# SegataLab/metamlst

Hardware: NVIDIA B200
Metric: aligned reads/s (score+pileup+consensus) (higher is better)
Workload: dtype int32/u8 (integer bit-plane arithmetic)

## Files before the change

include/mmlst.h:

```cpp
#ifndef MMLST_H
#define MMLST_H

#include <stddef.h>
#include <stdint.h>

#ifdef __cplusplus
extern "C" {
#endif

#define MMLST_VERSION 200

enum {
    MMLST_OK = 0,
    MMLST_E_ARG = -1,
    MMLST_E_CUDA = -2,
    MMLST_E_IO = -3,
    MMLST_E_BAM = -4,
    MMLST_E_UNSORTED = -5,
    MMLST_E_PAIRED = -6,
    MMLST_E_RANGE = -7,
    MMLST_E_NOMEM = -8
};

typedef struct mmlst_ctx mmlst_ctx;

const char* mmlst_last_error(void);
int mmlst_version(void);
int mmlst_device_count(void);

int mmlst_create(int device, mmlst_ctx** out);
void mmlst_destroy(mmlst_ctx* ctx);
void* mmlst_stream(mmlst_ctx* ctx);
int mmlst_sync(mmlst_ctx* ctx);

void* mmlst_pinned_alloc(size_t bytes);
void mmlst_pinned_free(void* p);

int mmlst_score_dev(const uint32_t* tid, const int16_t* as0, const uint8_t* xm3, const uint16_t* qlen,
                    const uint32_t* orig_idx, uint64_t n_rec, uint64_t idx_base,
                    const uint8_t* allow, const uint32_t* locus_of, uint32_t n_ref,
                    int minscore, int max_xm, int min_read_len,
                    int64_t* sum_as, uint32_t* n_hit, uint32_t* first_idx, uint64_t* counters, void* stream);

int mmlst_build_runs(const uint32_t* tid, uint64_t n_rec, uint32_t* run_tid, uint32_t* run_start, uint32_t* chunk_run,
                     uint32_t* n_runs);
int mmlst_score_runs_dev(const uint32_t* run_tid, const uint32_t* run_start, uint32_t n_runs, const uint32_t* chunk_run,
                         const int16_t* as0, const uint8_t* xm3, const uint16_t* qlen, const uint32_t* orig_idx,
                         uint64_t n_rec, uint64_t idx_base, const uint8_t* allow, uint32_t n_ref,
                         int minscore, int max_xm, int min_read_len,
                         int64_t* sum_as, uint32_t* n_hit, uint32_t* first_idx, uint64_t* counters, void* stream);
int mmlst_chunk_qlen(const uint16_t* qlen, uint64_t n_rec, uint16_t* chunk_qlen, int* uniform);
int mmlst_score_runs_qc_dev(const uint32_t* run_tid, const uint32_t* run_start, uint32_t n_runs, const uint32_t* chunk_run,
                            const uint16_t* chunk_qlen, const int16_t* as0, const uint8_t* xm3, const uint32_t* orig_idx,
                            uint64_t n_rec, uint64_t idx_base, const uint8_t* allow, uint32_t n_ref,
                            int minscore, int max_xm, int min_read_len,
                            int64_t* sum_as, uint32_t* n_hit, uint32_t* first_idx, uint64_t* counters, void* stream);
#define MMLST_SCORE_VARIANT_DEFAULT 6
int mmlst_set_score_variant(int variant);
#define MMLST_SCORE_L2_HINTS_DEFAULT 1
int mmlst_set_score_l2_hints(int on);
int mmlst_debug_timeline(uint64_t* dev_buf);
#define MMLST_SCORE_GRID_DEFAULT 8
int mmlst_set_score_grid_scale(int eighths);
int mmlst_as_untransform_dev(int16_t* as0, const uint8_t* xm3, uint64_t n, int coeff, void* stream);
int mmlst_expand_chunk_qlen_dev(const uint16_t* chunk_qlen, uint64_t n_rec, uint16_t* qlen, void* stream);
int mmlst_expand_runs_dev(const uint32_t* run_tid, const uint32_t* run_start, uint32_t n_runs, const uint32_t* chunk_run,
                          uint64_t n_rec, uint32_t* tid, void* stream);

uint64_t mmlst_coverage_table_slots(uint64_t n_names_upper_bound);
int mmlst_coverage_dev(const uint32_t* tid, const int16_t* as0, const uint8_t* xm3, const uint16_t* qlen,
                       const uint32_t* orig_idx, const uint64_t* qhash, uint64_t n_rec, uint64_t idx_base,
                       const uint8_t* allow, const uint32_t* locus_of, uint32_t n_ref, int minscore, int max_xm,
                       int min_read_len, void* table, uint64_t table_slots, uint64_t* cov, void* stream);

typedef struct {
    int32_t pos;
    uint32_t row_off;
    uint16_t reflen;
    int16_t as_named;
    uint8_t xm_named;
    uint8_t pad;
    uint16_t nw;
} mmlst_prec;

typedef struct {
    uint32_t rec_begin, rec_end;
    uint32_t col_base, contig_len;
    uint32_t plane_delta;
    uint32_t reserved[3];
} mmlst_chunk;

uint32_t mmlst_chunk_records(uint64_t n_rec);

int mmlst_pileup_dev(const mmlst_prec* recs, const uint32_t* planes,
                     const mmlst_chunk* chunks, uint32_t n_chunks, uint32_t max_row_words,
                     int minscore, int max_xm, uint32_t* counts, uint32_t total_cols, int impl, void* stream);

int mmlst_depth_cap(const uint32_t* tid, const int32_t* pos, const uint32_t* reflen, uint64_t n, uint32_t maxcnt,
                    uint32_t sentinel_nodes, uint8_t* admitted);

int mmlst_consensus_dev(const uint32_t* counts, const uint8_t* dbseq, const uint32_t* col_off, uint32_t n_loci,
                        uint32_t mincov, uint8_t* cons, uint32_t* holes, uint32_t* snps, void* stream);

#define MMLST_SELECT_WARP_DEFAULT 0
int mmlst_set_select_warp_finalize(int on);
#define MMLST_SELECT_CONSUME 1u
#define MMLST_SELECT_SCRATCH_CLEAN 2u
#define MMLST_SELECT_LOCAL 4u
int mmlst_select_dev(int64_t* sum_as, uint32_t* n_hit, uint32_t* first_idx, const uint32_t* locus_rows, const uint32_t* locus_start,
                     const uint32_t* allele_num, uint32_t n_ref, const uint32_t* species_of_locus, const uint32_t* genes_in_db,
                     uint32_t n_loci, uint32_t n_species, int penalty, int nloci_pct, const uint64_t* contig_start,
                     const uint32_t* ref_len, const uint64_t* db_off, uint32_t chunk_records, void* scratch, size_t scratch_bytes,
                     uint32_t* header, uint32_t* chosen_tid, uint32_t* chosen_species, uint32_t* col_off, uint64_t* db_start,
                     mmlst_chunk* chunks, uint32_t max_chunks, uint32_t flags, uint64_t* counters,
                     uint32_t* chosen_first , void* stream);
int mmlst_set_pdl(int on);
int mmlst_pileup_indirect_dev(const mmlst_prec* recs, const uint32_t* planes, const mmlst_chunk* chunks, const uint32_t* header,
                              uint32_t max_row_words, int minscore, int max_xm, uint32_t* counts, int impl, void* stream);
int mmlst_pileup_consensus_indirect_dev(const mmlst_prec* recs, const uint32_t* planes, const mmlst_chunk* chunks, const uint32_t* header,
                                        uint32_t max_row_words, int minscore, int max_xm, uint32_t* counts, const uint8_t* db_ascii,
                                        const uint64_t* db_start, const uint32_t* col_off, uint32_t max_loci, uint32_t mincov, uint8_t* cons,
                                        uint32_t* holes, uint32_t* snps, uint32_t flags, uint32_t* ticket, void* stream);
#define MMLST_CONSENSUS_CONSUME 1u
int mmlst_consensus_indirect_dev(uint32_t* counts, const uint8_t* db_ascii, const uint64_t* db_start, const uint32_t* col_off,
                                 uint32_t max_loci, const uint32_t* header, uint32_t mincov, uint8_t* cons, uint32_t* holes,
                                 uint32_t* snps, uint32_t flags, void* stream);

int mmlst_xchg_publish_dev(const void* block, uint32_t bytes, const uint64_t* peer_base, uint32_t rank, uint32_t world,
                           uint64_t half_stride, uint64_t slot_stride, uint64_t flag_off, const uint64_t* epoch, void* stream);
int mmlst_xchg_await_dev(void* local_base, uint32_t bytes, uint32_t world, uint64_t half_stride, uint64_t slot_stride,
                         uint64_t flag_off, void* out_all, uint64_t* epoch, uint32_t* ticket, uint32_t* status, void* stream);

typedef struct mmlst_comm mmlst_comm;
int mmlst_comm_unique_id(uint8_t* id128);
int mmlst_comm_create(const uint8_t* id128, int rank, int world, int device, mmlst_comm** out);
void mmlst_comm_destroy(mmlst_comm* comm);
int mmlst_allreduce(mmlst_comm* comm, int64_t* score_block, size_t score_words, uint32_t* first_idx, size_t n_ref, uint32_t* counts, size_t n_counts,
                    void* stream);

int mmlst_hamming_min_dev(const uint32_t* db_hi, const uint32_t* db_lo, const uint16_t* row_len, uint32_t n_rows,
                          uint32_t W, const uint32_t* q_hi, const uint32_t* q_lo, const uint16_t* q_len, uint32_t n_q,
                          const uint32_t* blocks, uint32_t n_blocks, uint32_t row_index_base,
                          unsigned long long* best, void* stream);
int mmlst_hamming_exact_dev(const uint32_t* db_hi, const uint32_t* db_lo, const uint16_t* row_len, uint32_t n_rows, uint32_t W,
                            const uint32_t* q_hi, const uint32_t* q_lo, const uint16_t* q_len, uint32_t n_q,
                            const uint32_t* blocks, uint32_t n_blocks, uint32_t row_index_base,
                            const uint32_t* xr_ids, const uint32_t* xr_x, const uint8_t* xr_bytes, uint32_t n_xr,
                            const uint32_t* xq_ids, const uint32_t* xq_x, const uint8_t* xq_bytes, uint32_t n_xq,
                            unsigned long long* best, void* stream);
int mmlst_hamming_min_dev2(const uint32_t* db_hi, const uint32_t* db_lo, const uint16_t* row_len, uint32_t n_rows,
                           uint32_t W, const uint32_t* q_hi, const uint32_t* q_lo, const uint16_t* q_len, uint32_t n_q,
                           const uint32_t* blocks, uint32_t n_blocks, uint32_t max_block_rows, uint32_t max_block_queries,
                           uint32_t row_index_base, unsigned long long* best, void* stream);

typedef struct {
    const uint8_t* bytes; uint64_t n_bytes;
    const uint64_t* table; uint32_t n_blocks;
    int32_t as_xm_coeff;
} mmlst_zstream;

typedef struct {
    const uint8_t* bytes; uint64_t n_bytes;
    const uint64_t* table; uint32_t n_blocks;
    const uint32_t* contig_block;
} mmlst_zpileup;

typedef struct {
    const uint32_t* tid; const int16_t* as0; const uint8_t* xm3; const uint16_t* qlen; const uint32_t* orig_idx;
    uint64_t n_rec;
    const mmlst_prec* p_recs;
    const uint32_t* planes; uint64_t n_prec; uint64_t n_plane_words; uint32_t max_row_words;
    const uint64_t* contig_start;
    uint32_t n_ref;
    uint32_t n_runs;
    const uint32_t* run_tid; const uint32_t* run_start; const uint32_t* chunk_run;
    const uint16_t* chunk_qlen;
    const mmlst_zstream* z;
    const mmlst_zpileup* zp;
} mmlst_soa;

typedef struct { int minscore, max_xm, min_read_len; } mmlst_score_params;

int mmlst_score(mmlst_ctx* ctx, const mmlst_soa* soa, const uint8_t* allow, const uint32_t* locus_of, uint32_t n_loci,
                const mmlst_score_params* prm, int64_t* sum_as, uint32_t* n_hit, uint32_t* first_idx, uint64_t* counters);

typedef struct {
    const uint32_t* locus_of; const uint32_t* allele_num; uint32_t n_ref;
    const uint32_t* species_of_locus; uint32_t n_loci;
    const uint32_t* genes_in_db; uint32_t n_species;
    const uint8_t* db_ascii; const uint64_t* db_off; const uint32_t* bam_ln;
} mmlst_index;
typedef struct { int minscore, max_xm, min_read_len, penalty, nloci_pct; uint32_t mincov; int pileup_impl; } mmlst_sample_params;
typedef struct {
    uint32_t n_chosen, error_bits, bad_len_tid, reserved;
    uint64_t total_reads, ignored_reads;
    uint32_t* chosen_tid; uint32_t* chosen_species; uint32_t* col_off;
    uint8_t* cons; uint64_t cons_capacity;
    uint32_t* holes; uint32_t* snps;
    int64_t* sum_as; uint32_t* n_hit; uint32_t* first_idx;
} mmlst_sample_result;
int mmlst_index_upload(mmlst_ctx* ctx, const mmlst_index* index);
int mmlst_sample(mmlst_ctx* ctx, const mmlst_soa* soa, const uint8_t* allow, const mmlst_sample_params* prm, mmlst_sample_result* res);

#define MMLST_COVERAGE_STREAM_RESIDENT 1u
int mmlst_coverage(mmlst_ctx* ctx, const mmlst_soa* soa, const uint64_t* qhash, const uint8_t* allow, const uint32_t* locus_of,
                   uint32_t n_loci, const mmlst_score_params* prm, uint32_t flags, uint64_t* cov);

int mmlst_pileup_consensus(mmlst_ctx* ctx, const mmlst_soa* soa, const uint32_t* chosen_tid, uint32_t n_loci,
                           const uint8_t* dbseq, const uint32_t* col_off, int minscore, int max_xm, uint32_t mincov,
                           int impl, uint32_t* counts, uint8_t* cons, uint32_t* holes, uint32_t* snps);

int mmlst_db_upload(mmlst_ctx* ctx, const uint32_t* db_hi, const uint32_t* db_lo, const uint16_t* row_len,
                    uint32_t n_rows, uint32_t W);
int mmlst_hamming_min(mmlst_ctx* ctx, const uint32_t* q_hi, const uint32_t* q_lo, const uint16_t* q_len, uint32_t n_q,
                      const uint32_t* blocks, uint32_t n_blocks, uint32_t* min_dist, uint32_t* argmin_row);
int mmlst_db_upload_x(mmlst_ctx* ctx, const uint32_t* db_hi, const uint32_t* db_lo, const uint16_t* row_len, uint32_t n_rows,
                      uint32_t W, const uint32_t* xr_ids, const uint32_t* xr_x, const uint8_t* xr_bytes, uint32_t n_xr);
int mmlst_hamming_min_x(mmlst_ctx* ctx, const uint32_t* q_hi, const uint32_t* q_lo, const uint16_t* q_len, uint32_t n_q,
                        const uint32_t* xq_ids, const uint32_t* xq_x, const uint8_t* xq_bytes, uint32_t n_xq,
                        const uint32_t* blocks, uint32_t n_blocks, uint32_t* min_dist, uint32_t* argmin_row);

size_t mmlst_hamming_tc_image_bytes(uint32_t n, uint32_t W, uint32_t tile_rows);
int mmlst_hamming_tc_expand_dev(const uint32_t* hi, const uint32_t* lo, const uint16_t* len, uint32_t n, uint32_t W, int db_tiled_layout,
                                uint32_t tile_rows, uint8_t* image, uint32_t* tile_maxlen, void* stream);
int mmlst_hamming_tc_search_dev(const uint8_t* q_image, const uint32_t* q_tile_maxlen, const uint16_t* q_len, uint32_t n_q,
                                const uint8_t* db_image, const uint32_t* db_tile_maxlen, const uint16_t* row_len, uint32_t n_rows,
                                uint32_t W, uint32_t row_index_base, unsigned long long* best, void* stream);

int mmlst_exact_match_dev(const uint32_t* db_hi, const uint32_t* db_lo, const uint16_t* row_len, uint32_t n_rows, uint32_t W,
                          const uint32_t* q_hi, const uint32_t* q_lo, const uint16_t* q_len, uint32_t n_q,
                          const uint32_t* blocks, uint32_t n_blocks, uint32_t max_block_rows, uint32_t row_index_base,
                          const uint32_t* row_key , const uint32_t* xr_ids, const uint8_t* xr_bytes, uint32_t n_xr,
                          const uint32_t* xq_ids, const uint8_t* xq_bytes, uint32_t n_xq, uint32_t* first_row, void* stream);
int mmlst_db_row_keys(mmlst_ctx* ctx, const uint32_t* row_key, uint32_t n_rows);
int mmlst_exact_match(mmlst_ctx* ctx, const uint32_t* q_hi, const uint32_t* q_lo, const uint16_t* q_len, uint32_t n_q,
                      const uint32_t* xq_ids, const uint8_t* xq_bytes, uint32_t n_xq,
                      const uint32_t* blocks, uint32_t n_blocks, uint32_t* first_row);

int mmlst_st_match_dev(const uint32_t* prof_start, const uint32_t* prof_allele, uint32_t n_st,
                       const uint32_t* q_alleles, const uint32_t* q_n, uint32_t l_max, uint32_t n_q,
                       uint32_t* count, uint32_t* best, uint32_t* n_best, uint32_t* out_idx, uint32_t max_out, void* stream);
int mmlst_profiles_upload(mmlst_ctx* ctx, const uint32_t* prof_start, const uint32_t* prof_allele, uint32_t n_st);
int mmlst_st_match(mmlst_ctx* ctx, const uint32_t* q_alleles, const uint32_t* q_n, uint32_t l_max, uint32_t n_q,
                   uint32_t* best, uint32_t* n_best, uint32_t* out_idx, uint32_t max_out);

int mmlst_inflate_raw(const uint8_t* in, size_t n, uint8_t* out, size_t out_capacity, size_t* produced);

typedef struct mmlst_bam mmlst_bam;
typedef struct {
    int minqual; uint32_t max_depth; uint32_t sentinel_nodes; int n_threads; int pinned; int assume_sorted;
    int want_qhash; int check_crc;
    int lenient_tags;
} mmlst_unpack_opts;
typedef struct {
    mmlst_soa soa;
    const uint64_t* qhash;
    const uint32_t* ref_len;
    const char* ref_names;
    const char* header_text;
    uint64_t n_dropped_by_cap, n_unmapped_flag;
    int presorted, minqual; uint32_t max_depth;
    double seconds[5];
    uint64_t n_untagged;
} mmlst_bam_info_t;
int mmlst_bam_unpack(const char* path, const mmlst_unpack_opts* opts , mmlst_bam** out);
int mmlst_bam_info(const mmlst_bam* bam, mmlst_bam_info_t* info);
void mmlst_bam_free(mmlst_bam* bam);

typedef struct mmlst_dev_bam mmlst_dev_bam;
typedef struct {
    const uint32_t* tid; const int16_t* as0; const uint8_t* xm3; const uint16_t* qlen; const uint32_t* orig_idx; const uint64_t* qhash;
    const uint32_t* run_tid; const uint32_t* run_start; const uint32_t* chunk_run; const uint16_t* chunk_qlen; uint32_t n_runs;
    const mmlst_prec* p_recs; const uint32_t* planes;
    uint64_t n_rec, n_prec, n_plane_words; uint32_t max_row_words;
    const uint64_t* contig_start;
    const uint32_t* ref_len;
    const char* ref_names;
    const char* header_text;
    uint32_t n_ref;
    uint64_t n_dropped_by_cap, n_unmapped_flag, n_bgzf_blocks, compressed_bytes, inflated_bytes;
    int presorted, minqual; uint32_t max_depth; int boundary_repairs;
    double seconds[8];
} mmlst_dev_bam_info_t;
int mmlst_bam_ingest(int device, const uint8_t* bam, size_t n_bytes, const mmlst_unpack_opts* opts, void* stream, mmlst_dev_bam** out);
int mmlst_dev_bam_info(const mmlst_dev_bam* bam, mmlst_dev_bam_info_t* info);
void mmlst_dev_bam_free(mmlst_dev_bam* bam);
int mmlst_ingest_trim(int device);

#ifdef __cplusplus
}
#endif
#endif
```

metamlst_b200/bam.py:

```python
from __future__ import annotations

import ctypes as C
import os
from typing import Optional

import numpy as np

from . import native, packing


class UnpackOpts(C.Structure):
    _fields_ = [("minqual", C.c_int), ("max_depth", C.c_uint32), ("sentinel_nodes", C.c_uint32), ("n_threads", C.c_int),
                ("pinned", C.c_int), ("assume_sorted", C.c_int), ("want_qhash", C.c_int), ("check_crc", C.c_int), ("lenient_tags", C.c_int)]


class BamInfo(C.Structure):
    _fields_ = [("soa", native.Soa), ("qhash", C.c_void_p), ("ref_len", C.c_void_p), ("ref_names", C.c_char_p),
                ("header_text", C.c_char_p), ("n_dropped_by_cap", C.c_uint64), ("n_unmapped_flag", C.c_uint64),
                ("presorted", C.c_int), ("minqual", C.c_int), ("max_depth", C.c_uint32), ("seconds", C.c_double * 5), ("n_untagged", C.c_uint64)]


class _Handle:
    def __init__(self, h):
        self.h = h

    def __del__(self):
        try:
            if self.h:
                native.lib().mmlst_bam_free(self.h)
                self.h = None
        except Exception:
            pass


def _view(addr: Optional[int], n: int, dtype) -> np.ndarray:
    dt = np.dtype(dtype)
    if not addr or n == 0:
        return np.zeros(0, dtype=dt)
    buf = (C.c_uint8 * (n * dt.itemsize)).from_address(addr)
    return np.frombuffer(buf, dtype=dt, count=n)


def unpack_bam(path: str, minqual: int = packing.DEFAULT_MINQUAL, max_depth: Optional[int] = packing.DEFAULT_MAX_DEPTH,
               presorted: bool = False, threads: int = 0, pinned: bool = True, want_qhash: bool = True,
               sentinel_nodes: int = 1, lenient_tags: bool = False) -> packing.SoaHost:
    lib = native.lib()
    o = UnpackOpts(int(minqual), int(max_depth or 0), int(sentinel_nodes), int(threads), 1 if pinned else 0,
                   1 if presorted else 0, 1 if want_qhash else 0, 1, 1 if lenient_tags else 0)
    h = C.c_void_p()
    native.check(lib.mmlst_bam_unpack(path.encode(), C.byref(o), C.byref(h)))
    keep = _Handle(h)
    info = BamInfo()
    native.check(lib.mmlst_bam_info(h, C.byref(info)))
    s = info.soa
    n, P, n_ref = int(s.n_rec), int(s.n_prec), int(s.n_ref)
    names = info.ref_names.decode("latin-1").split("\n") if n_ref else []
    soa = packing.SoaHost(
        names, _view(info.ref_len, n_ref, np.uint32).astype(np.int32),
        _view(s.tid, n, np.uint32), _view(s.as0, n, np.int16), _view(s.xm3, n, np.uint8), _view(s.qlen, n, np.uint16),
        _view(s.orig_idx, n, np.uint32) if s.orig_idx else None,
        _view(s.p_recs, P, packing.PREC_DTYPE), _view(s.planes, int(s.n_plane_words), np.uint32), int(s.max_row_words),
        _view(s.contig_start, n_ref + 1, np.uint64), int(info.minqual), int(info.max_depth), int(info.n_dropped_by_cap))
    if s.run_tid:
        nr = int(s.n_runs)
        soa.run_tid, soa.run_start = _view(s.run_tid, nr, np.uint32), _view(s.run_start, nr + 1, np.uint32)
        soa.chunk_run = _view(s.chunk_run, (n + 255) // 256, np.uint32)
        soa.chunk_qlen = _view(s.chunk_qlen, (n + 255) // 256, np.uint16) if s.chunk_qlen else None
        if nr > 0.125 * n:
            soa.run_tid = soa.run_start = soa.chunk_run = soa.chunk_qlen = None
    soa.qhash = _view(info.qhash, 2 * n, np.uint64).reshape(n, 2) if info.qhash else None
    soa.header_text = (info.header_text or b"").decode("latin-1")
    soa.unpack_seconds = dict(zip(("read", "inflate", "parse", "sort", "pack"), [float(x) for x in info.seconds]))
    soa.lenient, soa.n_untagged = bool(lenient_tags), int(info.n_untagged)
    soa._keep = (keep,)
    return soa


class DevBamInfo(C.Structure):
    _fields_ = [("tid", C.c_void_p), ("as0", C.c_void_p), ("xm3", C.c_void_p), ("qlen", C.c_void_p), ("orig_idx", C.c_void_p), ("qhash", C.c_void_p),
                ("run_tid", C.c_void_p), ("run_start", C.c_void_p), ("chunk_run", C.c_void_p), ("chunk_qlen", C.c_void_p), ("n_runs", C.c_uint32),
                ("p_recs", C.c_void_p), ("planes", C.c_void_p),
                ("n_rec", C.c_uint64), ("n_prec", C.c_uint64), ("n_plane_words", C.c_uint64), ("max_row_words", C.c_uint32),
                ("contig_start", C.c_void_p), ("ref_len", C.c_void_p), ("ref_names", C.c_char_p), ("header_text", C.c_char_p), ("n_ref", C.c_uint32),
                ("n_dropped_by_cap", C.c_uint64), ("n_unmapped_flag", C.c_uint64), ("n_bgzf_blocks", C.c_uint64), ("compressed_bytes", C.c_uint64),
                ("inflated_bytes", C.c_uint64), ("presorted", C.c_int), ("minqual", C.c_int), ("max_depth", C.c_uint32), ("boundary_repairs", C.c_int),
                ("seconds", C.c_double * 8)]


class _DevHandle:
    def __init__(self, h):
        self.h = h

    def __del__(self):
        try:
            if self.h:
                native.lib().mmlst_dev_bam_free(self.h)
                self.h = None
        except Exception:
            pass


class _DevArray:

    def __init__(self, addr: int, n: int, typestr: str, keep):
        self.__cuda_array_interface__ = {"shape": (n,), "typestr": typestr, "data": (addr, False), "version": 2, "strides": None}
        self._keep = keep


class PinnedPool:

    def __init__(self):
        import threading
        self._lock = threading.Lock()
        self._free = []

    def get(self, n: int):
        import torch
        with self._lock:
            best = None
            for i, t in enumerate(self._free):
                if t.numel() >= n and (best is None or t.numel() < self._free[best].numel()):
                    best = i
            if best is not None:
                return self._free.pop(best)
        return torch.empty(max(int(n * 1.25), 1 << 20), dtype=torch.uint8, pin_memory=torch.cuda.is_available())

    def put(self, t) -> None:
        base = getattr(t, "_pool_base", None)
        if base is not None:
            with self._lock:
                if len(self._free) < 16:
                    self._free.append(base)


POOL = PinnedPool()


def read_pinned(path: str, pool: Optional[PinnedPool] = None):
    import torch
    size = os.path.getsize(path)
    if pool is not None:
        base = pool.get(size)
    else:
        base = torch.empty(max(size, 1), dtype=torch.uint8, pin_memory=torch.cuda.is_available())
    with open(path, "rb") as fh:
        got = fh.readinto(memoryview(base.numpy())[:size]) if size else 0
    if got != size:
        raise IOError("short read on %s" % path)
    view = base[:size]
    if pool is not None:
        view._pool_base = base
    return view


def ingest_bam(source, device=0, minqual: int = packing.DEFAULT_MINQUAL, max_depth: Optional[int] = packing.DEFAULT_MAX_DEPTH,
               presorted: bool = False, want_qhash: bool = True, sentinel_nodes: int = 1, check_crc: bool = False):
    import torch
    from . import streams
    dev = torch.device("cuda", device) if isinstance(device, int) else torch.device(device)
    data = read_pinned(source) if isinstance(source, str) else source
    addr = data.data_ptr() if hasattr(data, "data_ptr") else data.ctypes.data
    nbytes = int(data.numel() if hasattr(data, "numel") else data.size)
    lib = native.lib()
    o = UnpackOpts(int(minqual), int(max_depth or 0), int(sentinel_nodes), 0, 1, 1 if presorted else 0, 1 if want_qhash else 0,
                  1 if check_crc else 0, 0)
    h = C.c_void_p()
    with torch.cuda.device(dev):
        stream = torch.cuda.current_stream(dev).cuda_stream
        native.check(lib.mmlst_bam_ingest(dev.index or 0, addr, nbytes, C.byref(o), stream, C.byref(h)))
    keep = _DevHandle(h)
    info = DevBamInfo()
    native.check(lib.mmlst_dev_bam_info(h, C.byref(info)))
    n, P, n_ref, nr = int(info.n_rec), int(info.n_prec), int(info.n_ref), int(info.n_runs)

    def t(addr_, count, typestr, dtype):
        if not addr_ or count == 0:
            return torch.zeros(0, dtype=dtype, device=dev)
        return torch.as_tensor(_DevArray(addr_, count, typestr, keep), device=dev)

    s = streams.DeviceStreams()
    s._keep = keep
    s.ref_names = info.ref_names.decode("latin-1").split("\n") if n_ref else []
    s.ref_lens = _view(info.ref_len, n_ref, np.uint32).astype(np.int32)
    s.header_text = (info.header_text or b"").decode("latin-1")
    s.minqual, s.max_depth, s.n_dropped = int(info.minqual), int(info.max_depth), int(info.n_dropped_by_cap)
    s.idx_base = 0
    s.tid, s.as0 = t(info.tid, n, "<i4", torch.int32), t(info.as0, n, "<i2", torch.int16)
    s.xm3, s.qlen = t(info.xm3, n, "|u1", torch.uint8), t(info.qlen, n, "<i2", torch.int16)
    s.orig_idx = t(info.orig_idx, n, "<i4", torch.int32) if info.orig_idx else None
    s.qhash = t(info.qhash, 2 * n, "<i8", torch.int64).view(n, 2) if (info.qhash and want_qhash) else None
    s.p_recs = t(info.p_recs, 4 * P, "<i4", torch.int32).view(P, 4)
    s.planes = t(info.planes, int(info.n_plane_words), "<i4", torch.int32)
    s.n_prec, s.max_row_words = P, int(info.max_row_words)
    s.contig_start = _view(info.contig_start, n_ref + 1, np.uint64).copy()
    s.run_tid = s.run_start = s.chunk_run = s.chunk_qlen = None
    if nr and nr <= 0.125 * n:
        s.run_tid, s.run_start = t(info.run_tid, nr, "<i4", torch.int32), t(info.run_start, nr + 1, "<i4", torch.int32)
        s.chunk_run = t(info.chunk_run, (n + 255) // 256, "<i4", torch.int32)
        s.chunk_qlen = t(info.chunk_qlen, (n + 255) // 256, "<i2", torch.int16) if info.chunk_qlen else None
    s.presorted = bool(info.presorted)
    s.ingest_seconds = dict(zip(("h2d", "inflate", "chain", "parse", "sort", "score_stream", "cap_compact", "pack"), [float(x) for x in info.seconds]))
    s.ingest_stats = {"bgzf_blocks": int(info.n_bgzf_blocks), "compressed_bytes": int(info.compressed_bytes), "inflated_bytes": int(info.inflated_bytes),
                      "boundary_repairs": int(info.boundary_repairs), "unmapped_flag": int(info.n_unmapped_flag)}
    return s
```

metamlst_b200/csrc/score_runs.cu:

```cuda
#include <stdlib.h>

#include "score_runs_kernels.cuh"


static int g_score_variant = -1;
static int score_variant() {
    if (g_score_variant < 0) {
        const char* e = getenv("MMLST_SCORE_VARIANT");
        g_score_variant = (e && e[0] >= '0' && e[0] <= '6' && !e[1]) ? e[0] - '0' : MMLST_SCORE_VARIANT_DEFAULT;
    }
    return g_score_variant;
}
extern "C" int mmlst_set_score_variant(int v) {
    const int prev = score_variant();
    if (v >= 0 && v <= 6) g_score_variant = v;
    return prev;
}

static int g_score_l2_hints = -1;
static int score_l2_hints() {
    if (g_score_l2_hints < 0) {
        const char* e = getenv("MMLST_SCORE_L2_HINTS");
        g_score_l2_hints = e ? (e[0] == '1') : MMLST_SCORE_L2_HINTS_DEFAULT;
    }
    return g_score_l2_hints;
}
extern "C" int mmlst_set_score_l2_hints(int on) {
    const int prev = score_l2_hints();
    if (on == 0 || on == 1) g_score_l2_hints = on;
    return prev;
}

static int g_score_grid8 = -1;
static int score_grid8() {
    if (g_score_grid8 < 0) {
        const char* e = getenv("MMLST_SCORE_GRID");
        const int v = e ? atoi(e) : 0;
        g_score_grid8 = (v >= 1 && v <= 64) ? v : MMLST_SCORE_GRID_DEFAULT;
    }
    return g_score_grid8;
}
extern "C" int mmlst_set_score_grid_scale(int eighths) {
    const int prev = score_grid8();
    if (eighths >= 1 && eighths <= 64) g_score_grid8 = eighths;
    return prev;
}

static int score_runs_launch(const uint32_t* run_tid, const uint32_t* run_start, uint32_t n_runs, const uint32_t* chunk_run,
                             const int16_t* as0, const uint8_t* xm3, const uint16_t* qlen, const uint16_t* chunk_qlen, const uint32_t* orig_idx,
                             uint64_t n_rec, uint64_t idx_base, const uint8_t* allow, uint32_t n_ref, int minscore,
                             int max_xm, int min_read_len, int64_t* sum_as, uint32_t* n_hit, uint32_t* first_idx,
                             uint64_t* counters, void* stream) {
    if (n_rec == 0) return MMLST_OK;
    if (!run_tid || !run_start || !chunk_run || !n_runs || !as0 || !xm3 || (!qlen && !chunk_qlen) || !allow || !sum_as || !n_hit || !first_idx || !counters) {
        mmlst_set_error("mmlst_score_runs_dev: null pointer");
        return MMLST_E_ARG;
    }
    if (n_rec >= 0xffffff00ull) { mmlst_set_error("mmlst_score_runs_dev: %llu records do not fit 32-bit run offsets", (unsigned long long)n_rec); return MMLST_E_RANGE; }
    if ((reinterpret_cast<uintptr_t>(as0) & 15) || (reinterpret_cast<uintptr_t>(xm3) & 7) || (!chunk_qlen && (reinterpret_cast<uintptr_t>(qlen) & 15)) ||
        (orig_idx && (reinterpret_cast<uintptr_t>(orig_idx) & 15))) {
        mmlst_set_error("mmlst_score_runs_dev: record arrays must be 16-byte aligned (as0/qlen/orig_idx), 8 (xm3)");
        return MMLST_E_ARG;
    }
    RunArgs a{run_tid, run_start, chunk_run, n_runs, as0, xm3, qlen, orig_idx, chunk_qlen, n_rec, idx_base, allow, n_ref, minscore, max_xm,
              min_read_len, reinterpret_cast<long long*>(sum_as), n_hit, first_idx, reinterpret_cast<unsigned long long*>(counters), score_l2_hints()};
    const uint64_t nchunks = n_rec >> 8;
    uint64_t want = (nchunks + 15) / 16;
    const int variant = score_variant();
    const cudaStream_t st = static_cast<cudaStream_t>(stream);
    const bool tma_ok = !orig_idx && !(reinterpret_cast<uintptr_t>(xm3) & 15);
    if (variant == 6 && tma_ok && chunk_qlen) {
        static int pair_resident_by_device[MMLST_MAX_DEVICES] = {0};
        int& pair_resident = pair_resident_by_device[mmlst_current_device()];
        const size_t smem = (kThreads / 32) * 2u * (4u * 768u + sizeof(uint64_t));
        if (!pair_resident) {
            CUDA_TRY(cudaFuncSetAttribute(score_runs_ring_pair_kernel, cudaFuncAttributeMaxDynamicSharedMemorySize, static_cast<int>(smem)));
            CUDA_TRY(cudaFuncSetAttribute(score_runs_ring_pair_kernel, cudaFuncAttributePreferredSharedMemoryCarveout, cudaSharedmemCarveoutMaxShared));
            int r = 0;
            if (cudaOccupancyMaxActiveBlocksPerMultiprocessor(&r, score_runs_ring_pair_kernel, kThreads, smem) != cudaSuccess || r < 1) r = 1;
            pair_resident = r;
        }
        const uint64_t cap = static_cast<uint64_t>(mmlst_num_sms()) * pair_resident * score_grid8() / 8;
        if (want > cap) want = cap;
        if (want < 1) want = 1;
        score_runs_ring_pair_kernel<<<static_cast<unsigned>(want), kThreads, smem, st>>>(a);
        CUDA_TRY(cudaGetLastError());
        return MMLST_OK;
    }
    if (variant >= 2 && tma_ok) {
        static int ring_resident_by_device[MMLST_MAX_DEVICES][4][8] = {{{0}}};
        int (&ring_resident)[4][8] = ring_resident_by_device[mmlst_current_device()];
        const int hint = a.l2_hints ? 1 : 0;
        const int q = (chunk_qlen ? 1 : 0) + 2 * hint;
        const int rv = variant == 6 ? 5 : variant;
        const RingCfg cfg = chunk_qlen ? (hint ? ring_config<true, true>(rv) : ring_config<true, false>(rv))
                                       : (hint ? ring_config<false, true>(rv) : ring_config<false, false>(rv));
        const size_t smem = (kThreads / 32) * static_cast<size_t>(cfg.ns) * (cfg.ch * (chunk_qlen ? 768u : 1280u) + sizeof(uint64_t));
        if (!ring_resident[q][rv]) {
            CUDA_TRY(cudaFuncSetAttribute(cfg.kern, cudaFuncAttributeMaxDynamicSharedMemorySize, static_cast<int>(smem)));
            CUDA_TRY(cudaFuncSetAttribute(cfg.kern, cudaFuncAttributePreferredSharedMemoryCarveout, cudaSharedmemCarveoutMaxShared));
            int r = 0;
            if (cudaOccupancyMaxActiveBlocksPerMultiprocessor(&r, cfg.kern, kThreads, smem) != cudaSuccess || r < 1) r = 1;
            ring_resident[q][rv] = r;
        }
        const uint64_t cap = static_cast<uint64_t>(mmlst_num_sms()) * ring_resident[q][rv];
        if (want > cap) want = cap;
        if (want < 1) want = 1;
        cfg.kern<<<static_cast<unsigned>(want), kThreads, smem, st>>>(a);
        CUDA_TRY(cudaGetLastError());
        return MMLST_OK;
    }
    static int resident_by_device[MMLST_MAX_DEVICES][8] = {{0}};
    int (&resident)[8] = resident_by_device[mmlst_current_device()];
    const int v = (orig_idx ? 1 : 0) + 2 * (variant == 1 ? 1 : 0) + (chunk_qlen ? 4 : 0);
    void (*const kerns[8])(const RunArgs) = {score_runs_kernel<false, false, false>, score_runs_kernel<true, false, false>,
                                             score_runs_kernel<false, true, false>, score_runs_kernel<true, true, false>,
                                             score_runs_kernel<false, false, true>, score_runs_kernel<true, false, true>,
                                             score_runs_kernel<false, true, true>, score_runs_kernel<true, true, true>};
    void (*kern)(const RunArgs) = kerns[v];
    if (!resident[v]) {
        if (cudaOccupancyMaxActiveBlocksPerMultiprocessor(&resident[v], kern, kThreads, 0) != cudaSuccess || resident[v] < 1) resident[v] = 3;
    }
    const uint64_t cap = static_cast<uint64_t>(mmlst_num_sms()) * resident[v];
    if (want > cap) want = cap;
    if (want < 1) want = 1;
    kern<<<static_cast<unsigned>(want), kThreads, 0, st>>>(a);
    CUDA_TRY(cudaGetLastError());
    return MMLST_OK;
}

extern "C" int mmlst_score_runs_dev(const uint32_t* run_tid, const uint32_t* run_start, uint32_t n_runs, const uint32_t* chunk_run,
                                    const int16_t* as0, const uint8_t* xm3, const uint16_t* qlen, const uint32_t* orig_idx,
                                    uint64_t n_rec, uint64_t idx_base, const uint8_t* allow, uint32_t n_ref, int minscore,
                                    int max_xm, int min_read_len, int64_t* sum_as, uint32_t* n_hit, uint32_t* first_idx,
                                    uint64_t* counters, void* stream) {
    if (n_rec && !qlen) { mmlst_set_error("mmlst_score_runs_dev: null pointer"); return MMLST_E_ARG; }
    return score_runs_launch(run_tid, run_start, n_runs, chunk_run, as0, xm3, qlen, nullptr, orig_idx, n_rec, idx_base, allow, n_ref, minscore,
                             max_xm, min_read_len, sum_as, n_hit, first_idx, counters, stream);
}

extern "C" int mmlst_score_runs_qc_dev(const uint32_t* run_tid, const uint32_t* run_start, uint32_t n_runs, const uint32_t* chunk_run,
                                       const uint16_t* chunk_qlen, const int16_t* as0, const uint8_t* xm3, const uint32_t* orig_idx,
                                       uint64_t n_rec, uint64_t idx_base, const uint8_t* allow, uint32_t n_ref, int minscore,
                                       int max_xm, int min_read_len, int64_t* sum_as, uint32_t* n_hit, uint32_t* first_idx,
                                       uint64_t* counters, void* stream) {
    if (n_rec && !chunk_qlen) { mmlst_set_error("mmlst_score_runs_qc_dev: null pointer"); return MMLST_E_ARG; }
    return score_runs_launch(run_tid, run_start, n_runs, chunk_run, as0, xm3, nullptr, chunk_qlen, orig_idx, n_rec, idx_base, allow, n_ref,
                             minscore, max_xm, min_read_len, sum_as, n_hit, first_idx, counters, stream);
}

extern "C" int mmlst_expand_chunk_qlen_dev(const uint16_t* chunk_qlen, uint64_t n_rec, uint16_t* qlen, void* stream) {
    if (n_rec == 0) return MMLST_OK;
    if (!chunk_qlen || !qlen) { mmlst_set_error("mmlst_expand_chunk_qlen_dev: null pointer"); return MMLST_E_ARG; }
    uint64_t blocks = (n_rec + 255) / 256;
    const uint64_t cap = static_cast<uint64_t>(mmlst_num_sms()) * 16;
    if (blocks > cap) blocks = cap;
    expand_chunk_qlen_kernel<<<static_cast<unsigned>(blocks), 256, 0, static_cast<cudaStream_t>(stream)>>>(chunk_qlen, n_rec, qlen);
    CUDA_TRY(cudaGetLastError());
    return MMLST_OK;
}

extern "C" int mmlst_expand_runs_dev(const uint32_t* run_tid, const uint32_t* run_start, uint32_t n_runs, const uint32_t* chunk_run,
                                     uint64_t n_rec, uint32_t* tid, void* stream) {
    if (n_rec == 0) return MMLST_OK;
    if (!run_tid || !run_start || !chunk_run || !n_runs || !tid) { mmlst_set_error("mmlst_expand_runs_dev: null pointer"); return MMLST_E_ARG; }
    uint64_t blocks = (n_rec + 255) / 256;
    const uint64_t cap = static_cast<uint64_t>(mmlst_num_sms()) * 16;
    if (blocks > cap) blocks = cap;
    expand_runs_kernel<<<static_cast<unsigned>(blocks), 256, 0, static_cast<cudaStream_t>(stream)>>>(run_tid, run_start, chunk_run, n_runs, n_rec, tid);
    CUDA_TRY(cudaGetLastError());
    return MMLST_OK;
}

namespace {
__global__ void __launch_bounds__(256) as_untransform_kernel(int16_t* __restrict__ as0, const uint8_t* __restrict__ xm3, uint64_t n, int coeff) {
    const uint64_t n8 = n >> 3;
    const uint64_t stride = static_cast<uint64_t>(gridDim.x) * blockDim.x;
    for (uint64_t i = static_cast<uint64_t>(blockIdx.x) * blockDim.x + threadIdx.x; i < n8; i += stride) {
        uint4 a = reinterpret_cast<uint4*>(as0)[i];
        const uint2 x = ld_stream_u2(xm3 + (i << 3));
        uint32_t aw[4] = {a.x, a.y, a.z, a.w};
        const uint32_t xw[2] = {x.x, x.y};
#pragma unroll
        for (int w = 0; w < 4; ++w) {
            const uint32_t xb = xw[w >> 1] >> ((w & 1) * 16);
            const int lo = static_cast<int16_t>(aw[w] & 0xffffu) - coeff * static_cast<int>(xb & 0xffu);
            const int hi = static_cast<int16_t>(aw[w] >> 16) - coeff * static_cast<int>((xb >> 8) & 0xffu);
            aw[w] = (static_cast<uint32_t>(lo) & 0xffffu) | (static_cast<uint32_t>(hi) << 16);
        }
        reinterpret_cast<uint4*>(as0)[i] = make_uint4(aw[0], aw[1], aw[2], aw[3]);
    }
    if (blockIdx.x == 0 && threadIdx.x == 0)
        for (uint64_t i = n8 << 3; i < n; ++i) as0[i] = static_cast<int16_t>(as0[i] - coeff * static_cast<int>(xm3[i]));
}
}

extern "C" int mmlst_as_untransform_dev(int16_t* as0, const uint8_t* xm3, uint64_t n, int coeff, void* stream) {
    if (n == 0 || coeff == 0) return MMLST_OK;
    if (!as0 || !xm3) { mmlst_set_error("mmlst_as_untransform_dev: null pointer"); return MMLST_E_ARG; }
    if ((reinterpret_cast<uintptr_t>(as0) & 15) || (reinterpret_cast<uintptr_t>(xm3) & 7)) { mmlst_set_error("mmlst_as_untransform_dev: as0 must be 16-byte aligned, xm3 8"); return MMLST_E_ARG; }
    uint64_t blocks = ((n >> 3) + 255) / 256;
    const uint64_t cap = static_cast<uint64_t>(mmlst_num_sms()) * 8;
    if (blocks > cap) blocks = cap;
    if (blocks < 1) blocks = 1;
    as_untransform_kernel<<<static_cast<unsigned>(blocks), 256, 0, static_cast<cudaStream_t>(stream)>>>(as0, xm3, n, coeff);
    CUDA_TRY(cudaGetLastError());
    return MMLST_OK;
}
```

metamlst_b200/csrc/score_runs_kernels.cuh:

```cuda
#pragma once
#include "common.cuh"

namespace {

constexpr int kThreads = 256;
constexpr uint32_t FULL = 0xffffffffu;

struct RunArgs {
    const uint32_t* run_tid; const uint32_t* run_start; const uint32_t* chunk_run; uint32_t n_runs;
    const int16_t* as0; const uint8_t* xm3; const uint16_t* qlen; const uint32_t* orig_idx;
    const uint16_t* chunk_qlen;
    uint64_t n_rec; uint64_t idx_base;
    const uint8_t* allow; uint32_t n_ref;
    int minscore, max_xm, min_read_len;
    long long* sum_as; uint32_t* n_hit; uint32_t* first_idx; unsigned long long* counters;
    int l2_hints;
};

__device__ __forceinline__ void flush_run(const RunArgs& a, uint32_t key, long long s, uint32_t c, uint32_t mn) {
    if (c) {
        atomicAdd(reinterpret_cast<unsigned long long*>(a.sum_as + key), static_cast<unsigned long long>(s));
        atomicAdd(a.n_hit + key, c);
        atomicMin(a.first_idx + key, mn);
    }
}

template <bool OIDX> struct Loaded;
template <> struct Loaded<false> { uint4 a8, q8; uint2 x8; uint32_t cq; };
template <> struct Loaded<true> { uint4 a8, q8; uint2 x8; uint32_t cq; uint4 oa, ob; };

template <bool OIDX, bool QC>
__device__ __forceinline__ Loaded<OIDX> load_chunk(const RunArgs& a, uint64_t base_lane) {
    Loaded<OIDX> L;
    L.a8 = ld_stream_u4(a.as0 + base_lane);
    L.x8 = ld_stream_u2(a.xm3 + base_lane);
    if constexpr (QC) { L.cq = __ldg(a.chunk_qlen + (base_lane >> 8)); L.q8 = make_uint4(0, 0, 0, 0); }
    else { L.q8 = ld_stream_u4(a.qlen + base_lane); L.cq = 0; }
    if constexpr (OIDX) { L.oa = ld_stream_u4(a.orig_idx + base_lane); L.ob = ld_stream_u4(a.orig_idx + base_lane + 4); }
    return L;
}

template <bool OIDX>
__device__ __forceinline__ uint32_t rec_index(const Loaded<OIDX>& L, uint32_t idx0, int k) {
    if constexpr (OIDX) {
        const uint32_t oi[8] = {L.oa.x, L.oa.y, L.oa.z, L.oa.w, L.ob.x, L.ob.y, L.ob.z, L.ob.w};
        return oi[k];
    } else {
        return idx0 + k;
    }
}

struct WarpRun {
    uint32_t r, key, end;
    bool al;
    long long s; uint32_t c, mn;
};

__device__ __forceinline__ void open_run(const RunArgs& a, WarpRun& w, uint32_t r) {
    w.r = r;
    if (r < a.n_runs) {
        w.key = __ldg(a.run_tid + r);
        w.end = __ldg(a.run_start + r + 1);
        w.al = (w.key < a.n_ref) && a.allow[w.key];
    } else {
        w.key = 0xffffffffu; w.end = 0xffffffffu; w.al = false;
    }
    w.s = 0; w.c = 0; w.mn = 0xffffffffu;
}

__device__ __forceinline__ void close_run(const RunArgs& a, WarpRun& w, uint32_t lane) {
    if (lane == 0 && w.al) flush_run(a, w.key, w.s, w.c, w.mn);
}

struct Thr {
    uint32_t as_T, as_TL;
    uint32_t ql_T, ql_TL;
    uint32_t xm_T, xm_TH;
    uint32_t h8;
};
constexpr uint32_t H16 = 0x80008000u, H8 = 0x80808080u;

__device__ __forceinline__ Thr make_thr(const RunArgs& a) {
    Thr t;
    const bool none = a.minscore > 32767 || a.min_read_len > 65535 || a.max_xm < 0;
    const uint32_t ts = static_cast<uint32_t>(max(a.minscore, -32768) + 32768) & 0xffffu;
    const uint32_t tq = static_cast<uint32_t>(min(max(a.min_read_len, 0), 65535));
    const uint32_t tx = static_cast<uint32_t>(min(max(a.max_xm, 0), 255));
    t.as_T = ts | (ts << 16); t.as_TL = t.as_T & ~H16;
    t.ql_T = tq | (tq << 16); t.ql_TL = t.ql_T & ~H16;
    t.xm_T = tx * 0x01010101u; t.xm_TH = t.xm_T | H8;
    t.h8 = none ? 0u : H8;
    return t;
}

template <bool OIDX, bool QC>
__device__ __forceinline__ void lane_pass(const Loaded<OIDX>& L, const Thr& t, int min_read_len, uint32_t& p_lo, uint32_t& p_hi) {
    const uint32_t aw[4] = {L.a8.x, L.a8.y, L.a8.z, L.a8.w};
    const uint32_t qw[4] = {L.q8.x, L.q8.y, L.q8.z, L.q8.w};
    uint32_t m[4];
#pragma unroll
    for (int w = 0; w < 4; ++w) {
        const uint32_t da = (aw[w] | H16) - t.as_TL;
        const uint32_t ga = (~aw[w] & ~t.as_T) | ((aw[w] ^ t.as_T) & da);
        if constexpr (QC) {
            m[w] = ga;
        } else {
            const uint32_t dq = (qw[w] | H16) - t.ql_TL;
            const uint32_t gq = (qw[w] & ~t.ql_T) | (~(qw[w] ^ t.ql_T) & dq);
            m[w] = ga & gq;
        }
    }
    const uint32_t b_lo = __byte_perm(m[0], m[1], 0x7531), b_hi = __byte_perm(m[2], m[3], 0x7531);
    const uint32_t x0 = L.x8.x, x1 = L.x8.y;
    const uint32_t d0 = t.xm_TH - (x0 & ~H8), d1 = t.xm_TH - (x1 & ~H8);
    const uint32_t g0 = (t.xm_T & ~x0) | (~(t.xm_T ^ x0) & d0), g1 = (t.xm_T & ~x1) | (~(t.xm_T ^ x1) & d1);
    p_lo = (b_lo & g0 & t.h8) >> 7;
    p_hi = (b_hi & g1 & t.h8) >> 7;
    if constexpr (QC) {
        if (static_cast<int>(L.cq) < min_read_len) { p_lo = 0; p_hi = 0; }
    }
}

template <bool OIDX>
__device__ __forceinline__ void lane_sums(const Loaded<OIDX>& L, uint32_t p_lo, uint32_t p_hi, uint32_t idx0, int& s, uint32_t& c, uint32_t& mn) {
    s = __dp2a_lo(static_cast<int>(L.a8.x), static_cast<int>(p_lo), 0);
    s = __dp2a_hi(static_cast<int>(L.a8.y), static_cast<int>(p_lo), s);
    s = __dp2a_lo(static_cast<int>(L.a8.z), static_cast<int>(p_hi), s);
    s = __dp2a_hi(static_cast<int>(L.a8.w), static_cast<int>(p_hi), s);
    c = __popc(p_lo | (p_hi << 1));
    if constexpr (OIDX) {
        mn = 0xffffffffu;
#pragma unroll
        for (int k = 0; k < 8; ++k) mn = (((k < 4 ? p_lo : p_hi) >> (8 * (k & 3))) & 1u) ? min(mn, rec_index<true>(L, idx0, k)) : mn;
    } else {
        const uint32_t k = p_lo ? (static_cast<uint32_t>(__ffs(p_lo)) - 1u) >> 3 : 4u + ((static_cast<uint32_t>(__ffs(p_hi)) - 1u) >> 3);
        mn = (p_lo | p_hi) ? idx0 + k : 0xffffffffu;
    }
}

template <bool OIDX, bool QC>
__device__ __forceinline__ void reduce_chunk(const RunArgs& a, const Thr& thr, WarpRun& w, const Loaded<OIDX>& L, uint64_t base, uint32_t lane,
                                             uint32_t& tot, uint32_t& ign) {
    constexpr uint32_t R = 8;
    const uint64_t rec0 = base + (lane << 3);
    const uint32_t idx0 = static_cast<uint32_t>(a.idx_base + rec0);
    uint32_t p_lo, p_hi;
    lane_pass<OIDX, QC>(L, thr, a.min_read_len, p_lo, p_hi);
    const uint64_t chunk_end = base + 256;
    if (chunk_end <= w.end) {
        if (w.al) {
            int s; uint32_t c, mn;
            lane_sums<OIDX>(L, p_lo, p_hi, idx0, s, c, mn);
            tot += R;
            ign += R - c;
            w.s += __reduce_add_sync(FULL, s);
            w.c += __reduce_add_sync(FULL, c);
            w.mn = min(w.mn, __reduce_min_sync(FULL, mn));
        }
        if (chunk_end == w.end) { close_run(a, w, lane); open_run(a, w, w.r + 1); }
        return;
    }
    uint64_t lo = base;
    while (lo < chunk_end) {
        const uint64_t hi = (w.end < chunk_end) ? static_cast<uint64_t>(w.end) : chunk_end;
        if (w.al) {
            const uint32_t klo = lo <= rec0 ? 0u : (lo - rec0 >= R ? R : static_cast<uint32_t>(lo - rec0));
            const uint32_t khi = hi <= rec0 ? 0u : (hi - rec0 >= R ? R : static_cast<uint32_t>(hi - rec0));
            const unsigned long long ones = 0x0101010101010101ull;
            const unsigned long long below_hi = khi >= 8 ? ~0ull : ((1ull << (8 * khi)) - 1ull);
            const unsigned long long below_lo = klo >= 8 ? ~0ull : ((1ull << (8 * klo)) - 1ull);
            const unsigned long long inm = khi > klo ? (below_hi & ~below_lo & ones) : 0ull;
            const uint32_t in_lo = static_cast<uint32_t>(inm), in_hi = static_cast<uint32_t>(inm >> 32);
            int s; uint32_t c, mn;
            lane_sums<OIDX>(L, p_lo & in_lo, p_hi & in_hi, idx0, s, c, mn);
            const uint32_t in = khi > klo ? khi - klo : 0u;
            tot += in;
            ign += in - c;
            w.s += __reduce_add_sync(FULL, s);
            w.c += __reduce_add_sync(FULL, c);
            w.mn = min(w.mn, __reduce_min_sync(FULL, mn));
        }
        if (hi == w.end) { close_run(a, w, lane); open_run(a, w, w.r + 1); }
        lo = hi;
    }
}

template <bool QC>
__device__ __forceinline__ void score_tail(const RunArgs& a, uint64_t nchunks, uint32_t lane, uint32_t& tot, uint32_t& ign) {
    uint32_t r = __ldg(a.chunk_run + nchunks);
    for (uint64_t i = (nchunks << 8) + lane; i < a.n_rec; i += 32) {
        while (r + 1 < a.n_runs && i >= a.run_start[r + 1]) ++r;
        const uint32_t key = a.run_tid[r];
        if (!((key < a.n_ref) && a.allow[key])) continue;
        ++tot;
        const int as = a.as0[i];
        const int ql = QC ? int(a.chunk_qlen[nchunks]) : int(a.qlen[i]);
        if ((as >= a.minscore) && (ql >= a.min_read_len) && (int(a.xm3[i]) <= a.max_xm)) {
            const uint32_t idx = a.orig_idx ? a.orig_idx[i] : static_cast<uint32_t>(a.idx_base + i);
            flush_run(a, key, as, 1u, idx);
        } else {
            ++ign;
        }
    }
}

template <bool OIDX, bool PIPE, bool QC>
__global__ void __launch_bounds__(kThreads, PIPE ? (OIDX ? 2 : 3) : (OIDX ? 3 : 4)) score_runs_kernel(const RunArgs a) {
    pdl_launch_dependents();
    const uint32_t lane = threadIdx.x & 31u;
    const uint64_t warp = (static_cast<uint64_t>(blockIdx.x) * blockDim.x + threadIdx.x) >> 5;
    const uint64_t nwarps = (static_cast<uint64_t>(gridDim.x) * blockDim.x) >> 5;
    const uint64_t nchunks = a.n_rec >> 8;
    const uint64_t per = (nchunks + nwarps - 1) / nwarps;
    const uint64_t c0 = warp * per;
    const uint64_t c1 = (c0 + per < nchunks) ? c0 + per : nchunks;
    uint32_t tot = 0, ign = 0;
    const Thr thr = make_thr(a);

    if (c0 < c1) {
        uint64_t ch = c0;
        Loaded<OIDX> A0, A1;
        bool have = ch + 1 < c1;
        if (have) { A0 = load_chunk<OIDX, QC>(a, (ch << 8) + (lane << 3)); A1 = load_chunk<OIDX, QC>(a, ((ch + 1) << 8) + (lane << 3)); }
        WarpRun w;
        open_run(a, w, __ldg(a.chunk_run + c0));
        Loaded<OIDX> B0, B1;
        if constexpr (!PIPE) {
            while (have) {
                reduce_chunk<OIDX, QC>(a, thr, w, A0, ch << 8, lane, tot, ign);
                reduce_chunk<OIDX, QC>(a, thr, w, A1, (ch + 1) << 8, lane, tot, ign);
                ch += 2;
                have = ch + 1 < c1;
                if (have) { A0 = load_chunk<OIDX, QC>(a, (ch << 8) + (lane << 3)); A1 = load_chunk<OIDX, QC>(a, ((ch + 1) << 8) + (lane << 3)); }
            }
        }
        while (have) {
            const bool moreB = ch + 3 < c1;
            if (moreB) { B0 = load_chunk<OIDX, QC>(a, ((ch + 2) << 8) + (lane << 3)); B1 = load_chunk<OIDX, QC>(a, ((ch + 3) << 8) + (lane << 3)); }
            reduce_chunk<OIDX, QC>(a, thr, w, A0, ch << 8, lane, tot, ign);
            reduce_chunk<OIDX, QC>(a, thr, w, A1, (ch + 1) << 8, lane, tot, ign);
            ch += 2;
            if (!moreB) break;
            have = ch + 3 < c1;
            if (have) { A0 = load_chunk<OIDX, QC>(a, ((ch + 2) << 8) + (lane << 3)); A1 = load_chunk<OIDX, QC>(a, ((ch + 3) << 8) + (lane << 3)); }
            reduce_chunk<OIDX, QC>(a, thr, w, B0, ch << 8, lane, tot, ign);
            reduce_chunk<OIDX, QC>(a, thr, w, B1, (ch + 1) << 8, lane, tot, ign);
            ch += 2;
        }
        if (ch < c1) {
            const uint64_t base = ch << 8;
            const Loaded<OIDX> L0 = load_chunk<OIDX, QC>(a, base + (lane << 3));
            reduce_chunk<OIDX, QC>(a, thr, w, L0, base, lane, tot, ign);
        }
        close_run(a, w, lane);
    }

    if (warp == nwarps - 1 && (a.n_rec & 255u)) score_tail<QC>(a, nchunks, lane, tot, ign);
    tot = __reduce_add_sync(FULL, tot);
    ign = __reduce_add_sync(FULL, ign);
    if (lane == 0 && tot) {
        atomicAdd(a.counters + 0, static_cast<unsigned long long>(tot));
        atomicAdd(a.counters + 1, static_cast<unsigned long long>(ign));
    }
}

struct WarpRunPF {
    uint32_t r, key, end;
    uint32_t nkey, nend;
    bool al;
    long long s; uint32_t c, mn;
};

template <bool HINT> __device__ __forceinline__ uint32_t tab_u32(const uint32_t* p, uint64_t pol) {
    if constexpr (HINT) return ld_table_u32(p, pol); else return __ldg(p);
}
template <bool HINT> __device__ __forceinline__ uint32_t tab_u16(const uint16_t* p, uint64_t pol) {
    if constexpr (HINT) return ld_table_u16(p, pol); else return __ldg(p);
}
template <bool HINT> __device__ __forceinline__ uint32_t tab_u8(const uint8_t* p, uint64_t pol) {
    if constexpr (HINT) return ld_table_u8(p, pol); else return *p;
}
template <bool HINT>
__device__ __forceinline__ void request_next_run(const RunArgs& a, WarpRunPF& w, uint64_t pol) {
    if (w.r + 1u < a.n_runs) { w.nkey = tab_u32<HINT>(a.run_tid + w.r + 1u, pol); w.nend = tab_u32<HINT>(a.run_start + w.r + 2u, pol); }
    else { w.nkey = 0xffffffffu; w.nend = 0xffffffffu; }
}
template <bool HINT>
__device__ __forceinline__ void open_run_pf(const RunArgs& a, WarpRunPF& w, uint32_t r, uint64_t pol) {
    w.r = r;
    if (r < a.n_runs) { w.key = tab_u32<HINT>(a.run_tid + r, pol); w.end = tab_u32<HINT>(a.run_start + r + 1u, pol); }
    else { w.key = 0xffffffffu; w.end = 0xffffffffu; }
    request_next_run<HINT>(a, w, pol);
    w.al = (w.key < a.n_ref) && tab_u8<HINT>(a.allow + w.key, pol);
    w.s = 0; w.c = 0; w.mn = 0xffffffffu;
}
template <bool HINT>
__device__ __forceinline__ void next_run_pf(const RunArgs& a, WarpRunPF& w, uint32_t lane, uint64_t pol) {
    if (lane == 0 && w.al) flush_run(a, w.key, w.s, w.c, w.mn);
    w.r += 1u; w.key = w.nkey; w.end = w.nend;
    request_next_run<HINT>(a, w, pol);
    w.al = (w.key < a.n_ref) && tab_u8<HINT>(a.allow + w.key, pol);
    w.s = 0; w.c = 0; w.mn = 0xffffffffu;
}

__device__ __forceinline__ uint32_t bytes_below(uint32_t k) { return k >= 4u ? 0xffffffffu : ((1u << (8u * k)) - 1u); }
__device__ __forceinline__ void segment_masks(uint32_t klo, uint32_t khi, uint32_t& in_lo, uint32_t& in_hi) {
    in_lo = bytes_below(min(khi, 4u)) & ~bytes_below(min(klo, 4u)) & 0x01010101u;
    in_hi = bytes_below(khi > 4u ? khi - 4u : 0u) & ~bytes_below(klo > 4u ? klo - 4u : 0u) & 0x01010101u;
}

__device__ __forceinline__ void lane_sums_pf(const Loaded<false>& L, uint32_t p_lo, uint32_t p_hi, int& s, uint32_t& c) {
    s = __dp2a_lo(static_cast<int>(L.a8.x), static_cast<int>(p_lo), 0);
    s = __dp2a_hi(static_cast<int>(L.a8.y), static_cast<int>(p_lo), s);
    s = __dp2a_lo(static_cast<int>(L.a8.z), static_cast<int>(p_hi), s);
    s = __dp2a_hi(static_cast<int>(L.a8.w), static_cast<int>(p_hi), s);
    c = __popc(p_lo | (p_hi << 1));
}
__device__ __forceinline__ uint32_t first_pass_index(uint32_t p_lo, uint32_t p_hi, uint32_t idx0) {
    const uint32_t k = p_lo ? (static_cast<uint32_t>(__ffs(p_lo)) - 1u) >> 3 : 4u + ((static_cast<uint32_t>(__ffs(p_hi)) - 1u) >> 3);
    return (p_lo | p_hi) ? idx0 + k : 0xffffffffu;
}

template <bool QC, bool HINT>
__device__ __forceinline__ void reduce_chunk_pf(const RunArgs& a, const Thr& thr, WarpRunPF& w, const Loaded<false>& L, uint32_t base, uint32_t lane,
                                                uint32_t& tot, uint32_t& ign, uint64_t pol) {
    constexpr uint32_t R = 8;
    const uint32_t idx0 = static_cast<uint32_t>(a.idx_base) + base + (lane << 3);
    uint32_t p_lo, p_hi;
    lane_pass<false, QC>(L, thr, a.min_read_len, p_lo, p_hi);
    const uint32_t chunk_end = base + 256u;
    if (chunk_end <= w.end) {
        if (w.al) {
            int s; uint32_t c;
            lane_sums_pf(L, p_lo, p_hi, s, c);
            tot += R;
            ign += R - c;
            w.s += __reduce_add_sync(FULL, s);
            w.c += __reduce_add_sync(FULL, c);
            if (w.mn == 0xffffffffu) w.mn = __reduce_min_sync(FULL, first_pass_index(p_lo, p_hi, idx0));
        }
        if (chunk_end == w.end) next_run_pf<HINT>(a, w, lane, pol);
        return;
    }
    const int lane0 = static_cast<int>(lane << 3);
    uint32_t lo = base;
    while (lo < chunk_end) {
        const uint32_t hi = min(w.end, chunk_end);
        if (w.al) {
            const uint32_t klo = static_cast<uint32_t>(min(max(static_cast<int>(lo - base) - lane0, 0), 8));
            const uint32_t khi = static_cast<uint32_t>(min(max(static_cast<int>(hi - base) - lane0, 0), 8));
            uint32_t in_lo, in_hi;
            segment_masks(klo, khi, in_lo, in_hi);
            int s; uint32_t c;
            lane_sums_pf(L, p_lo & in_lo, p_hi & in_hi, s, c);
            const uint32_t in = khi - klo;
            tot += in;
            ign += in - c;
            w.s += __reduce_add_sync(FULL, s);
            w.c += __reduce_add_sync(FULL, c);
            if (w.mn == 0xffffffffu) w.mn = __reduce_min_sync(FULL, first_pass_index(p_lo & in_lo, p_hi & in_hi, idx0));
        }
        if (hi == w.end) next_run_pf<HINT>(a, w, lane, pol);
        lo = hi;
    }
}

template <bool QC, int NS, int CH, int MINB, bool HINT>
__global__ void __launch_bounds__(kThreads, MINB) score_runs_ring_kernel(const RunArgs a) {
    pdl_launch_dependents();
    extern __shared__ __align__(128) uint8_t ring_raw[];
    constexpr uint32_t AS_B = CH * 512u, QL_B = QC ? 0u : CH * 512u, XM_B = CH * 256u;
    constexpr uint32_t STAGE_B = AS_B + QL_B + XM_B;
    constexpr uint32_t CH_B = STAGE_B / CH;
    constexpr int NW = kThreads / 32;
    const uint32_t lane = threadIdx.x & 31u, wid = threadIdx.x >> 5;
    uint8_t* const my = ring_raw + wid * (NS * STAGE_B);
    uint64_t* const bars = reinterpret_cast<uint64_t*>(ring_raw + NW * NS * STAGE_B) + wid * NS;
    if (threadIdx.x == 0) {
        uint64_t* all = reinterpret_cast<uint64_t*>(ring_raw + NW * NS * STAGE_B);
        for (int i = 0; i < NW * NS; ++i) mbar_init(all + i, 1);
        fence_mbar_init();
    }
    __syncthreads();

    const uint64_t warp = (static_cast<uint64_t>(blockIdx.x) * blockDim.x + threadIdx.x) >> 5;
    const uint64_t nwarps = (static_cast<uint64_t>(gridDim.x) * blockDim.x) >> 5;
    const uint64_t nchunks = a.n_rec >> 8;
    const uint64_t per = (nchunks + nwarps - 1) / nwarps;
    const uint64_t c0 = warp * per;
    const uint64_t c1 = (c0 + per < nchunks) ? c0 + per : nchunks;
    uint32_t tot = 0, ign = 0;
    const Thr thr = make_thr(a);
    const uint64_t pol_s = HINT ? l2_policy(1) : 0ull, pol_t = HINT ? l2_policy(2) : 0ull;

    if (c0 < c1) {
        const uint32_t ngroups = static_cast<uint32_t>((c1 - c0 + CH - 1) / CH);
        auto issue = [&](uint32_t g, int stage) {
            const uint64_t ch = c0 + static_cast<uint64_t>(g) * CH;
            const uint32_t nch = (c1 - ch < CH) ? static_cast<uint32_t>(c1 - ch) : static_cast<uint32_t>(CH);
            uint8_t* st = my + stage * STAGE_B;
            mbar_expect_tx(bars + stage, nch * CH_B);
            if constexpr (HINT) {
                bulk_g2s_hint(st, a.as0 + (ch << 8), nch * 512u, bars + stage, pol_s);
                if constexpr (!QC) bulk_g2s_hint(st + AS_B, a.qlen + (ch << 8), nch * 512u, bars + stage, pol_s);
                bulk_g2s_hint(st + AS_B + QL_B, a.xm3 + (ch << 8), nch * 256u, bars + stage, pol_s);
            } else {
                bulk_g2s(st, a.as0 + (ch << 8), nch * 512u, bars + stage);
                if constexpr (!QC) bulk_g2s(st + AS_B, a.qlen + (ch << 8), nch * 512u, bars + stage);
                bulk_g2s(st + AS_B + QL_B, a.xm3 + (ch << 8), nch * 256u, bars + stage);
            }
        };
        if (lane == 0) {
            const uint32_t pre = ngroups < static_cast<uint32_t>(NS) ? ngroups : static_cast<uint32_t>(NS);
            for (uint32_t g = 0; g < pre; ++g) issue(g, static_cast<int>(g));
        }
        WarpRunPF w;
        open_run_pf<HINT>(a, w, tab_u32<HINT>(a.chunk_run + c0, pol_t), pol_t);
        uint32_t phase = 0;
        int stage = 0;
        for (uint32_t g = 0; g < ngroups; ++g) {
            const uint64_t ch = c0 + static_cast<uint64_t>(g) * CH;
            const uint32_t nch = (c1 - ch < CH) ? static_cast<uint32_t>(c1 - ch) : static_cast<uint32_t>(CH);
            mbar_wait(bars + stage, (phase >> stage) & 1u);
            phase ^= 1u << stage;
            const uint8_t* st = my + stage * STAGE_B;
#pragma unroll
            for (uint32_t k = 0; k < static_cast<uint32_t>(CH); ++k) {
                if (k < nch) {
                    Loaded<false> L;
                    L.a8 = *reinterpret_cast<const uint4*>(st + k * 512u + lane * 16u);
                    L.x8 = *reinterpret_cast<const uint2*>(st + AS_B + QL_B + k * 256u + lane * 8u);
                    if constexpr (QC) { L.q8 = make_uint4(0, 0, 0, 0); L.cq = tab_u16<HINT>(a.chunk_qlen + ch + k, pol_t); }
                    else { L.q8 = *reinterpret_cast<const uint4*>(st + AS_B + k * 512u + lane * 16u); L.cq = 0; }
                    if (k + 1u == nch) {
                        __syncwarp();
                        if (lane == 0 && g + NS < ngroups) issue(g + NS, stage);
                    }
                    reduce_chunk_pf<QC, HINT>(a, thr, w, L, static_cast<uint32_t>((ch + k) << 8), lane, tot, ign, pol_t);
                }
            }
            stage = (stage + 1 == NS) ? 0 : stage + 1;
        }
        if (lane == 0 && w.al) flush_run(a, w.key, w.s, w.c, w.mn);
    }

    if (warp == nwarps - 1 && (a.n_rec & 255u)) score_tail<QC>(a, nchunks, lane, tot, ign);
    tot = __reduce_add_sync(FULL, tot);
    ign = __reduce_add_sync(FULL, ign);
    if (lane == 0 && tot) {
        atomicAdd(a.counters + 0, static_cast<unsigned long long>(tot));
        atomicAdd(a.counters + 1, static_cast<unsigned long long>(ign));
    }
}

__device__ __forceinline__ void reduce_pair_pf(const RunArgs& a, const Thr& thr, WarpRunPF& w, const Loaded<false>& La, const Loaded<false>& Lb,
                                               uint32_t base, uint32_t lane, uint32_t& tot, uint32_t& ign, uint64_t pol) {
    if (base + 512u > w.end) {
        reduce_chunk_pf<true, false>(a, thr, w, La, base, lane, tot, ign, pol);
        reduce_chunk_pf<true, false>(a, thr, w, Lb, base + 256u, lane, tot, ign, pol);
        return;
    }
    if (w.al) {
        uint32_t pa_lo, pa_hi, pb_lo, pb_hi;
        lane_pass<false, true>(La, thr, a.min_read_len, pa_lo, pa_hi);
        lane_pass<false, true>(Lb, thr, a.min_read_len, pb_lo, pb_hi);
        int s = __dp2a_lo(static_cast<int>(La.a8.x), static_cast<int>(pa_lo), 0);
        s = __dp2a_hi(static_cast<int>(La.a8.y), static_cast<int>(pa_lo), s);
        s = __dp2a_lo(static_cast<int>(La.a8.z), static_cast<int>(pa_hi), s);
        s = __dp2a_hi(static_cast<int>(La.a8.w), static_cast<int>(pa_hi), s);
        s = __dp2a_lo(static_cast<int>(Lb.a8.x), static_cast<int>(pb_lo), s);
        s = __dp2a_hi(static_cast<int>(Lb.a8.y), static_cast<int>(pb_lo), s);
        s = __dp2a_lo(static_cast<int>(Lb.a8.z), static_cast<int>(pb_hi), s);
        s = __dp2a_hi(static_cast<int>(Lb.a8.w), static_cast<int>(pb_hi), s);
        const uint32_t c = __popc(pa_lo | (pa_hi << 1) | (pb_lo << 2) | (pb_hi << 3));
        tot += 16u;
        ign += 16u - c;
        w.s += __reduce_add_sync(FULL, s);
        w.c += __reduce_add_sync(FULL, c);
        if (w.mn == 0xffffffffu) {
            const uint32_t idx0 = static_cast<uint32_t>(a.idx_base) + base + (lane << 3);
            const uint32_t ma = first_pass_index(pa_lo, pa_hi, idx0);
            w.mn = __reduce_min_sync(FULL, ma != 0xffffffffu ? ma : first_pass_index(pb_lo, pb_hi, idx0 + 256u));
        }
    }
    if (base + 512u == w.end) next_run_pf<false>(a, w, lane, pol);
}

__global__ void __launch_bounds__(kThreads, 4) score_runs_ring_pair_kernel(const RunArgs a) {
    pdl_launch_dependents();
    extern __shared__ __align__(128) uint8_t ring_raw[];
    constexpr int NS = 2;
    constexpr uint32_t CH = 4, AS_B = CH * 512u, XM_B = CH * 256u, STAGE_B = AS_B + XM_B, CH_B = STAGE_B / CH;
    constexpr int NW = kThreads / 32;
    const uint32_t lane = threadIdx.x & 31u, wid = threadIdx.x >> 5;
    uint8_t* const my = ring_raw + wid * (NS * STAGE_B);
    uint64_t* const bars = reinterpret_cast<uint64_t*>(ring_raw + NW * NS * STAGE_B) + wid * NS;
    if (threadIdx.x == 0) {
        uint64_t* all = reinterpret_cast<uint64_t*>(ring_raw + NW * NS * STAGE_B);
        for (int i = 0; i < NW * NS; ++i) mbar_init(all + i, 1);
        fence_mbar_init();
    }
    __syncthreads();

    const uint64_t warp = (static_cast<uint64_t>(blockIdx.x) * blockDim.x + threadIdx.x) >> 5;
    const uint64_t nwarps = (static_cast<uint64_t>(gridDim.x) * blockDim.x) >> 5;
    const uint64_t nchunks = a.n_rec >> 8;
    const uint64_t per = (nchunks + nwarps - 1) / nwarps;
    const uint64_t c0 = warp * per;
    const uint64_t c1 = (c0 + per < nchunks) ? c0 + per : nchunks;
    uint32_t tot = 0, ign = 0;
    const Thr thr = make_thr(a);

    if (c0 < c1) {
        const uint32_t ngroups = static_cast<uint32_t>((c1 - c0 + CH - 1) / CH);
        auto issue = [&](uint32_t g, int stage) {
            const uint64_t ch = c0 + static_cast<uint64_t>(g) * CH;
            const uint32_t nch = (c1 - ch < CH) ? static_cast<uint32_t>(c1 - ch) : CH;
            uint8_t* st = my + stage * STAGE_B;
            mbar_expect_tx(bars + stage, nch * CH_B);
            if (a.l2_hints) {
                const uint64_t pol_s = l2_policy(1);
                bulk_g2s_hint(st, a.as0 + (ch << 8), nch * 512u, bars + stage, pol_s);
                bulk_g2s_hint(st + AS_B, a.xm3 + (ch << 8), nch * 256u, bars + stage, pol_s);
            } else {
                bulk_g2s(st, a.as0 + (ch << 8), nch * 512u, bars + stage);
                bulk_g2s(st + AS_B, a.xm3 + (ch << 8), nch * 256u, bars + stage);
            }
        };
        if (lane == 0) {
            const uint32_t pre = ngroups < static_cast<uint32_t>(NS) ? ngroups : static_cast<uint32_t>(NS);
            for (uint32_t g = 0; g < pre; ++g) issue(g, static_cast<int>(g));
        }
        WarpRunPF w;
        open_run_pf<false>(a, w, __ldg(a.chunk_run + c0), 0ull);
        uint32_t phase = 0;
        int stage = 0;
        auto load = [&](const uint8_t* st, uint32_t k, uint64_t ch) {
            Loaded<false> L;
            L.a8 = *reinterpret_cast<const uint4*>(st + k * 512u + lane * 16u);
            L.x8 = *reinterpret_cast<const uint2*>(st + AS_B + k * 256u + lane * 8u);
            L.q8 = make_uint4(0, 0, 0, 0);
            L.cq = __ldg(a.chunk_qlen + ch + k);
            return L;
        };
        for (uint32_t g = 0; g < ngroups; ++g) {
            const uint64_t ch = c0 + static_cast<uint64_t>(g) * CH;
            const uint32_t nch = (c1 - ch < CH) ? static_cast<uint32_t>(c1 - ch) : CH;
            mbar_wait(bars + stage, (phase >> stage) & 1u);
            phase ^= 1u << stage;
            const uint8_t* st = my + stage * STAGE_B;
#pragma unroll
            for (uint32_t k = 0; k < CH; k += 2) {
                if (k < nch) {
                    const bool two = k + 1u < nch;
                    const Loaded<false> La = load(st, k, ch);
                    Loaded<false> Lb = La;
                    if (two) Lb = load(st, k + 1u, ch);
                    if (k + 2u >= nch) {
                        __syncwarp();
                        if (lane == 0 && g + NS < ngroups) issue(g + NS, stage);
                    }
                    const uint32_t base = static_cast<uint32_t>((ch + k) << 8);
                    if (two) reduce_pair_pf(a, thr, w, La, Lb, base, lane, tot, ign, 0ull);
                    else reduce_chunk_pf<true, false>(a, thr, w, La, base, lane, tot, ign, 0ull);
                }
            }
            stage = (stage + 1 == NS) ? 0 : stage + 1;
        }
        if (lane == 0 && w.al) flush_run(a, w.key, w.s, w.c, w.mn);
    }

    if (warp == nwarps - 1 && (a.n_rec & 255u)) score_tail<true>(a, nchunks, lane, tot, ign);
    tot = __reduce_add_sync(FULL, tot);
    ign = __reduce_add_sync(FULL, ign);
    if (lane == 0 && tot) {
        atomicAdd(a.counters + 0, static_cast<unsigned long long>(tot));
        atomicAdd(a.counters + 1, static_cast<unsigned long long>(ign));
    }
}

struct RingCfg { void (*kern)(const RunArgs); uint32_t ch, ns; };
template <bool QC, bool HINT>
inline RingCfg ring_config(int variant) {
    if constexpr (QC) {
        switch (variant) {
            case 3: return {score_runs_ring_kernel<true, 3, 4, 3, HINT>, 4, 3};
            case 4: return {score_runs_ring_kernel<true, 2, 8, 2, HINT>, 8, 2};
            case 5: return {score_runs_ring_kernel<true, 2, 4, 4, HINT>, 4, 2};
            default: return {score_runs_ring_kernel<true, 4, 2, 4, HINT>, 2, 4};
        }
    } else {
        switch (variant) {
            case 3: case 4: case 5: return {score_runs_ring_kernel<false, 2, 4, 2, HINT>, 4, 2};
            default: return {score_runs_ring_kernel<false, 3, 2, 3, HINT>, 2, 3};
        }
    }
}

__global__ void __launch_bounds__(256) expand_runs_kernel(const uint32_t* __restrict__ run_tid, const uint32_t* __restrict__ run_start,
                                                          const uint32_t* __restrict__ chunk_run, uint32_t n_runs, uint64_t n_rec,
                                                          uint32_t* __restrict__ tid) {
    const uint64_t stride = static_cast<uint64_t>(gridDim.x) * blockDim.x;
    for (uint64_t i = static_cast<uint64_t>(blockIdx.x) * blockDim.x + threadIdx.x; i < n_rec; i += stride) {
        uint32_t r = __ldg(chunk_run + (i >> 8));
        while (r + 1 < n_runs && i >= __ldg(run_start + r + 1)) ++r;
        tid[i] = __ldg(run_tid + r);
    }
}

__global__ void __launch_bounds__(256) expand_chunk_qlen_kernel(const uint16_t* __restrict__ chunk_qlen, uint64_t n_rec, uint16_t* __restrict__ qlen) {
    const uint64_t stride = static_cast<uint64_t>(gridDim.x) * blockDim.x;
    for (uint64_t i = static_cast<uint64_t>(blockIdx.x) * blockDim.x + threadIdx.x; i < n_rec; i += stride) qlen[i] = __ldg(chunk_qlen + (i >> 8));
}

}
```

metamlst_b200/native.py:

```python
from __future__ import annotations

import ctypes as C
import os

_HERE = os.path.dirname(os.path.abspath(__file__))
LIB_PATH = os.path.join(_HERE, "libmmlst.so")


class MmlstError(RuntimeError):
    def __init__(self, code: int, msg: str):
        super().__init__("libmmlst error %d: %s" % (code, msg))
        self.code = code


E_ARG, E_CUDA, E_IO, E_BAM, E_UNSORTED, E_PAIRED, E_RANGE, E_NOMEM = -1, -2, -3, -4, -5, -6, -7, -8


class Chunk(C.Structure):
    _fields_ = [("rec_begin", C.c_uint32), ("rec_end", C.c_uint32), ("col_base", C.c_uint32), ("contig_len", C.c_uint32),
                ("plane_delta", C.c_uint32), ("reserved", C.c_uint32 * 3)]


class Soa(C.Structure):
    _fields_ = [("tid", C.c_void_p), ("as0", C.c_void_p), ("xm3", C.c_void_p), ("qlen", C.c_void_p), ("orig_idx", C.c_void_p),
                ("n_rec", C.c_uint64),
                ("p_recs", C.c_void_p),
                ("planes", C.c_void_p), ("n_prec", C.c_uint64), ("n_plane_words", C.c_uint64), ("max_row_words", C.c_uint32),
                ("contig_start", C.c_void_p), ("n_ref", C.c_uint32),
                ("n_runs", C.c_uint32), ("run_tid", C.c_void_p), ("run_start", C.c_void_p), ("chunk_run", C.c_void_p),
                ("chunk_qlen", C.c_void_p), ("z", C.c_void_p), ("zp", C.c_void_p)]


class ZStream(C.Structure):
    _fields_ = [("bytes", C.c_void_p), ("n_bytes", C.c_uint64), ("table", C.c_void_p), ("n_blocks", C.c_uint32), ("as_xm_coeff", C.c_int32)]


class ZPileup(C.Structure):
    _fields_ = [("bytes", C.c_void_p), ("n_bytes", C.c_uint64), ("table", C.c_void_p), ("n_blocks", C.c_uint32), ("contig_block", C.c_void_p)]


class ScoreParams(C.Structure):
    _fields_ = [("minscore", C.c_int), ("max_xm", C.c_int), ("min_read_len", C.c_int)]


class Index(C.Structure):
    _fields_ = [("locus_of", C.c_void_p), ("allele_num", C.c_void_p), ("n_ref", C.c_uint32),
                ("species_of_locus", C.c_void_p), ("n_loci", C.c_uint32),
                ("genes_in_db", C.c_void_p), ("n_species", C.c_uint32),
                ("db_ascii", C.c_void_p), ("db_off", C.c_void_p), ("bam_ln", C.c_void_p)]


class SampleParams(C.Structure):
    _fields_ = [("minscore", C.c_int), ("max_xm", C.c_int), ("min_read_len", C.c_int), ("penalty", C.c_int), ("nloci_pct", C.c_int),
                ("mincov", C.c_uint32), ("pileup_impl", C.c_int)]


class SampleResult(C.Structure):
    _fields_ = [("n_chosen", C.c_uint32), ("error_bits", C.c_uint32), ("bad_len_tid", C.c_uint32), ("reserved", C.c_uint32),
                ("total_reads", C.c_uint64), ("ignored_reads", C.c_uint64),
                ("chosen_tid", C.c_void_p), ("chosen_species", C.c_void_p), ("col_off", C.c_void_p),
                ("cons", C.c_void_p), ("cons_capacity", C.c_uint64),
                ("holes", C.c_void_p), ("snps", C.c_void_p),
                ("sum_as", C.c_void_p), ("n_hit", C.c_void_p), ("first_idx", C.c_void_p)]


EXPORTS = {
    "mmlst_last_error": (C.c_char_p, []),
    "mmlst_version": (C.c_int, []),
    "mmlst_device_count": (C.c_int, []),
    "mmlst_create": (C.c_int, [C.c_int, C.POINTER(C.c_void_p)]),
    "mmlst_destroy": (None, [C.c_void_p]),
    "mmlst_stream": (C.c_void_p, [C.c_void_p]),
    "mmlst_sync": (C.c_int, [C.c_void_p]),
    "mmlst_pinned_alloc": (C.c_void_p, [C.c_size_t]),
    "mmlst_pinned_free": (None, [C.c_void_p]),
    "mmlst_score_dev": (C.c_int, [C.c_void_p] * 5 + [C.c_uint64, C.c_uint64, C.c_void_p, C.c_void_p, C.c_uint32,
                                  C.c_int, C.c_int, C.c_int, C.c_void_p, C.c_void_p, C.c_void_p, C.c_void_p, C.c_void_p]),
    "mmlst_build_runs": (C.c_int, [C.c_void_p, C.c_uint64, C.c_void_p, C.c_void_p, C.c_void_p, C.POINTER(C.c_uint32)]),
    "mmlst_score_runs_dev": (C.c_int, [C.c_void_p, C.c_void_p, C.c_uint32] + [C.c_void_p] * 5 + [C.c_uint64, C.c_uint64, C.c_void_p, C.c_uint32,
                                       C.c_int, C.c_int, C.c_int, C.c_void_p, C.c_void_p, C.c_void_p, C.c_void_p, C.c_void_p]),
    "mmlst_chunk_qlen": (C.c_int, [C.c_void_p, C.c_uint64, C.c_void_p, C.POINTER(C.c_int)]),
    "mmlst_score_runs_qc_dev": (C.c_int, [C.c_void_p, C.c_void_p, C.c_uint32] + [C.c_void_p] * 5 + [C.c_uint64, C.c_uint64, C.c_void_p, C.c_uint32,
                                          C.c_int, C.c_int, C.c_int, C.c_void_p, C.c_void_p, C.c_void_p, C.c_void_p, C.c_void_p]),
    "mmlst_expand_chunk_qlen_dev": (C.c_int, [C.c_void_p, C.c_uint64, C.c_void_p, C.c_void_p]),
    "mmlst_inflate_raw": (C.c_int, [C.c_void_p, C.c_size_t, C.c_void_p, C.c_size_t, C.POINTER(C.c_size_t)]),
    "mmlst_set_score_variant": (C.c_int, [C.c_int]),
    "mmlst_set_score_l2_hints": (C.c_int, [C.c_int]),
    "mmlst_set_score_grid_scale": (C.c_int, [C.c_int]),
    "mmlst_debug_timeline": (C.c_int, [C.c_void_p]),
    "mmlst_set_select_warp_finalize": (C.c_int, [C.c_int]),
    "mmlst_as_untransform_dev": (C.c_int, [C.c_void_p, C.c_void_p, C.c_uint64, C.c_int, C.c_void_p]),
    "mmlst_set_pdl": (C.c_int, [C.c_int]),
    "mmlst_expand_runs_dev": (C.c_int, [C.c_void_p, C.c_void_p, C.c_uint32, C.c_void_p, C.c_uint64, C.c_void_p, C.c_void_p]),
    "mmlst_coverage_table_slots": (C.c_uint64, [C.c_uint64]),
    "mmlst_coverage_dev": (C.c_int, [C.c_void_p] * 6 + [C.c_uint64, C.c_uint64, C.c_void_p, C.c_void_p, C.c_uint32, C.c_int, C.c_int,
                                     C.c_int, C.c_void_p, C.c_uint64, C.c_void_p, C.c_void_p]),
    "mmlst_coverage": (C.c_int, [C.c_void_p, C.POINTER(Soa), C.c_void_p, C.c_void_p, C.c_void_p, C.c_uint32, C.POINTER(ScoreParams),
                                 C.c_uint32, C.c_void_p]),
    "mmlst_pileup_dev": (C.c_int, [C.c_void_p] * 3 + [C.c_uint32, C.c_uint32, C.c_int, C.c_int, C.c_void_p, C.c_uint32,
                                   C.c_int, C.c_void_p]),
    "mmlst_consensus_dev": (C.c_int, [C.c_void_p, C.c_void_p, C.c_void_p, C.c_uint32, C.c_uint32, C.c_void_p, C.c_void_p,
                                      C.c_void_p, C.c_void_p]),
    "mmlst_hamming_min_dev": (C.c_int, [C.c_void_p, C.c_void_p, C.c_void_p, C.c_uint32, C.c_uint32, C.c_void_p, C.c_void_p,
                                        C.c_void_p, C.c_uint32, C.c_void_p, C.c_uint32, C.c_uint32, C.c_void_p, C.c_void_p]),
    "mmlst_hamming_min_dev2": (C.c_int, [C.c_void_p, C.c_void_p, C.c_void_p, C.c_uint32, C.c_uint32, C.c_void_p, C.c_void_p,
                                         C.c_void_p, C.c_uint32, C.c_void_p, C.c_uint32, C.c_uint32, C.c_uint32, C.c_uint32,
                                         C.c_void_p, C.c_void_p]),
    "mmlst_select_dev": (C.c_int, [C.c_void_p] * 6 + [C.c_uint32, C.c_void_p, C.c_void_p, C.c_uint32, C.c_uint32, C.c_int, C.c_int,
                                   C.c_void_p, C.c_void_p, C.c_void_p, C.c_uint32, C.c_void_p, C.c_size_t] + [C.c_void_p] * 6 +
                         [C.c_uint32, C.c_uint32, C.c_void_p, C.c_void_p, C.c_void_p]),
    "mmlst_pileup_indirect_dev": (C.c_int, [C.c_void_p] * 4 + [C.c_uint32, C.c_int, C.c_int, C.c_void_p, C.c_int, C.c_void_p]),
    "mmlst_consensus_indirect_dev": (C.c_int, [C.c_void_p] * 4 + [C.c_uint32, C.c_void_p, C.c_uint32, C.c_void_p, C.c_void_p, C.c_void_p,
                                                C.c_uint32, C.c_void_p]),
    "mmlst_pileup_consensus_indirect_dev": (C.c_int, [C.c_void_p] * 4 + [C.c_uint32, C.c_int, C.c_int, C.c_void_p, C.c_void_p, C.c_void_p, C.c_void_p, C.c_uint32,
                                                      C.c_uint32, C.c_void_p, C.c_void_p, C.c_void_p, C.c_uint32, C.c_void_p, C.c_void_p]),
    "mmlst_chunk_records": (C.c_uint32, [C.c_uint64]),
    "mmlst_xchg_publish_dev": (C.c_int, [C.c_void_p, C.c_uint32, C.c_void_p, C.c_uint32, C.c_uint32, C.c_uint64, C.c_uint64, C.c_uint64,
                                         C.c_void_p, C.c_void_p]),
    "mmlst_xchg_await_dev": (C.c_int, [C.c_void_p, C.c_uint32, C.c_uint32, C.c_uint64, C.c_uint64, C.c_uint64, C.c_void_p, C.c_void_p,
                                       C.c_void_p, C.c_void_p, C.c_void_p]),
    "mmlst_depth_cap": (C.c_int, [C.c_void_p, C.c_void_p, C.c_void_p, C.c_uint64, C.c_uint32, C.c_uint32, C.c_void_p]),
    "mmlst_score": (C.c_int, [C.c_void_p, C.POINTER(Soa), C.c_void_p, C.c_void_p, C.c_uint32, C.POINTER(ScoreParams),
                              C.c_void_p, C.c_void_p, C.c_void_p, C.c_void_p]),
    "mmlst_pileup_consensus": (C.c_int, [C.c_void_p, C.POINTER(Soa), C.c_void_p, C.c_uint32, C.c_void_p, C.c_void_p, C.c_int,
                                         C.c_int, C.c_uint32, C.c_int, C.c_void_p, C.c_void_p, C.c_void_p, C.c_void_p]),
    "mmlst_db_upload": (C.c_int, [C.c_void_p, C.c_void_p, C.c_void_p, C.c_void_p, C.c_uint32, C.c_uint32]),
    "mmlst_db_upload_x": (C.c_int, [C.c_void_p, C.c_void_p, C.c_void_p, C.c_void_p, C.c_uint32, C.c_uint32, C.c_void_p, C.c_void_p,
                                    C.c_void_p, C.c_uint32]),
    "mmlst_hamming_min_x": (C.c_int, [C.c_void_p, C.c_void_p, C.c_void_p, C.c_void_p, C.c_uint32, C.c_void_p, C.c_void_p, C.c_void_p,
                                      C.c_uint32, C.c_void_p, C.c_uint32, C.c_void_p, C.c_void_p]),
    "mmlst_hamming_exact_dev": (C.c_int, [C.c_void_p, C.c_void_p, C.c_void_p, C.c_uint32, C.c_uint32, C.c_void_p, C.c_void_p, C.c_void_p,
                                          C.c_uint32, C.c_void_p, C.c_uint32, C.c_uint32, C.c_void_p, C.c_void_p, C.c_void_p, C.c_uint32,
                                          C.c_void_p, C.c_void_p, C.c_void_p, C.c_uint32, C.c_void_p, C.c_void_p]),
    "mmlst_exact_match_dev": (C.c_int, [C.c_void_p, C.c_void_p, C.c_void_p, C.c_uint32, C.c_uint32, C.c_void_p, C.c_void_p, C.c_void_p, C.c_uint32,
                                        C.c_void_p, C.c_uint32, C.c_uint32, C.c_uint32, C.c_void_p, C.c_void_p, C.c_void_p, C.c_uint32, C.c_void_p,
                                        C.c_void_p, C.c_uint32, C.c_void_p, C.c_void_p]),
    "mmlst_db_row_keys": (C.c_int, [C.c_void_p, C.c_void_p, C.c_uint32]),
    "mmlst_exact_match": (C.c_int, [C.c_void_p, C.c_void_p, C.c_void_p, C.c_void_p, C.c_uint32, C.c_void_p, C.c_void_p, C.c_uint32, C.c_void_p,
                                    C.c_uint32, C.c_void_p]),
    "mmlst_st_match_dev": (C.c_int, [C.c_void_p, C.c_void_p, C.c_uint32, C.c_void_p, C.c_void_p, C.c_uint32, C.c_uint32, C.c_void_p, C.c_void_p,
                                     C.c_void_p, C.c_void_p, C.c_uint32, C.c_void_p]),
    "mmlst_profiles_upload": (C.c_int, [C.c_void_p, C.c_void_p, C.c_void_p, C.c_uint32]),
    "mmlst_st_match": (C.c_int, [C.c_void_p, C.c_void_p, C.c_void_p, C.c_uint32, C.c_uint32, C.c_void_p, C.c_void_p, C.c_void_p, C.c_uint32]),
    "mmlst_bam_unpack": (C.c_int, [C.c_char_p, C.c_void_p, C.POINTER(C.c_void_p)]),
    "mmlst_bam_info": (C.c_int, [C.c_void_p, C.c_void_p]),
    "mmlst_bam_free": (None, [C.c_void_p]),
    "mmlst_hamming_min": (C.c_int, [C.c_void_p, C.c_void_p, C.c_void_p, C.c_void_p, C.c_uint32, C.c_void_p, C.c_uint32,
                                    C.c_void_p, C.c_void_p]),
    "mmlst_hamming_tc_image_bytes": (C.c_size_t, [C.c_uint32, C.c_uint32, C.c_uint32]),
    "mmlst_hamming_tc_expand_dev": (C.c_int, [C.c_void_p, C.c_void_p, C.c_void_p, C.c_uint32, C.c_uint32, C.c_int, C.c_uint32, C.c_void_p, C.c_void_p, C.c_void_p]),
    "mmlst_hamming_tc_search_dev": (C.c_int, [C.c_void_p, C.c_void_p, C.c_void_p, C.c_uint32, C.c_void_p, C.c_void_p, C.c_void_p, C.c_uint32, C.c_uint32,
                                              C.c_uint32, C.c_void_p, C.c_void_p]),
    "mmlst_ingest_trim": (C.c_int, [C.c_int]),
    "mmlst_comm_unique_id": (C.c_int, [C.c_void_p]),
    "mmlst_comm_create": (C.c_int, [C.c_void_p, C.c_int, C.c_int, C.c_int, C.POINTER(C.c_void_p)]),
    "mmlst_comm_destroy": (None, [C.c_void_p]),
    "mmlst_allreduce": (C.c_int, [C.c_void_p, C.c_void_p, C.c_size_t, C.c_void_p, C.c_size_t, C.c_void_p, C.c_size_t, C.c_void_p]),
    "mmlst_bam_ingest": (C.c_int, [C.c_int, C.c_void_p, C.c_size_t, C.c_void_p, C.c_void_p, C.POINTER(C.c_void_p)]),
    "mmlst_dev_bam_info": (C.c_int, [C.c_void_p, C.c_void_p]),
    "mmlst_dev_bam_free": (None, [C.c_void_p]),
    "mmlst_index_upload": (C.c_int, [C.c_void_p, C.c_void_p]),
    "mmlst_sample": (C.c_int, [C.c_void_p, C.c_void_p, C.c_void_p, C.c_void_p, C.c_void_p]),
}

_lib = None
SELECT_CONSUME, SELECT_SCRATCH_CLEAN, SELECT_LOCAL, CONSENSUS_CONSUME, COVERAGE_STREAM_RESIDENT = 1, 2, 4, 1, 1


def lib() -> C.CDLL:
    global _lib
    if _lib is None:
        if not os.path.exists(LIB_PATH):
            raise ImportError("%s is missing: run `python -c 'import __graft_entry__ as g; g.build()'` "
                              "(metamlst_b200 has no CPU fallback)" % LIB_PATH)
        l = C.CDLL(LIB_PATH)
        for name, (res, args) in EXPORTS.items():
            f = getattr(l, name)
            f.restype = res
            f.argtypes = args
        _lib = l
    return _lib


def check(rc: int) -> None:
    if rc != 0:
        raise MmlstError(rc, lib().mmlst_last_error().decode(errors="replace"))


def ptr(x) -> int:
    if x is None:
        return 0
    if hasattr(x, "data_ptr"):
        return x.data_ptr()
    return x.ctypes.data


class Context:

    def __init__(self, device: int = 0):
        self._h = C.c_void_p()
        check(lib().mmlst_create(device, C.byref(self._h)))
        self.device = device

    @property
    def handle(self):
        return self._h

    def close(self):
        if self._h:
            lib().mmlst_destroy(self._h)
            self._h = C.c_void_p()

    def __del__(self):
        try:
            self.close()
        except Exception:
            pass
```

metamlst_b200/pipeline.py:

```python
from __future__ import annotations

import os
from typing import Callable, Dict, List, Optional, Sequence, Tuple

import numpy as np
import torch

from . import api, dist, native

def build_chunks(contig_start: np.ndarray, chosen_tid: Sequence[int], col_off: np.ndarray) -> np.ndarray:
    out = []
    total = sum(int(contig_start[t + 1]) - int(contig_start[t]) for t in chosen_tid)
    CHUNK_RECORDS = int(native.lib().mmlst_chunk_records(total))
    for l, t in enumerate(chosen_tid):
        r0, r1 = int(contig_start[t]), int(contig_start[t + 1])
        for b in range(r0, r1, CHUNK_RECORDS):
            out.append((b, min(r1, b + CHUNK_RECORDS), int(col_off[l]), int(col_off[l + 1] - col_off[l]), 0, 0, 0, 0))
    return np.asarray(out, dtype=np.uint32).reshape(-1, 8)


class DevicePipeline:
    def __init__(self, streams, index: api.AlleleIndex, dbseq_of: Callable[[int], str], minscore: int = 80, max_xM: int = 5,
                 min_read_len: int = 50, penalty: int = 100, species_filter: Optional[str] = None, mincov: int = 1,
                 impl: int = 0, idx_base: int = 0, group=None, nloci: int = 100, genes_in_db: Optional[Dict[str, int]] = None,
                 db_ascii: Optional[np.ndarray] = None, db_off: Optional[np.ndarray] = None, exchange: str = "allreduce",
                 use_runs: Optional[bool] = None):
        self.s = streams
        self._use_runs_arg, self._idx_base_arg = use_runs, idx_base
        self.index = index
        self.dbseq_of = dbseq_of
        self.minscore, self.max_xM, self.min_read_len, self.penalty = int(minscore), api.check_max_xm(max_xM), int(min_read_len), int(penalty)
        self.mincov, self.impl = int(mincov), int(impl)
        self.idx_base = int(idx_base) if idx_base else int(getattr(streams, "idx_base", 0) or 0)
        self.group = group
        self.dist = torch.distributed.is_available() and torch.distributed.is_initialized() and torch.distributed.get_world_size() > 1
        if exchange not in ("allreduce", "gather", "p2p"):
            raise ValueError("exchange must be 'allreduce', 'gather' or 'p2p'")
        self.owner = self.dist and exchange in ("gather", "p2p")
        self.p2p = self.dist and exchange == "p2p"
        self.world = torch.distributed.get_world_size() if self.dist else 1
        dev = streams.as0.device
        self.dev = dev
        self.use_runs = bool(use_runs) if use_runs is not None else getattr(streams, "run_tid", None) is not None
        self.use_qc = self.use_runs and getattr(streams, "chunk_qlen", None) is not None
        n_ref = len(index.ref_names)
        self.n_ref = n_ref
        self.allow = torch.from_numpy(index.allow_mask(species_filter)).to(dev)
        self.locus_of = torch.from_numpy(index.locus_of.astype(np.int32)).to(dev)
        self.max_cols = int(np.sort(np.asarray(streams.ref_lens))[::-1][: index.n_loci].sum())
        w_hit, w_cnt = (n_ref + 1) // 2, (self.max_cols * 5 + 8 + 1) // 2
        self.zblock = torch.zeros(n_ref + 2 + w_hit + w_cnt, dtype=torch.int64, device=dev)
        self.zscore = self.zblock[: n_ref + 2 + w_hit]
        self.sum_as = self.zblock[:n_ref]
        self.counters = self.zblock[n_ref:n_ref + 2]
        self.n_hit = self.zblock[n_ref + 2:n_ref + 2 + w_hit].view(torch.int32)[:n_ref]
        self.counts = self.zblock[n_ref + 2 + w_hit:].view(torch.int32)[: self.max_cols * 5 + 8]
        self.first_idx = torch.zeros(n_ref, dtype=torch.int32, device=dev)
        self._db_cache: Dict[Tuple[int, ...], tuple] = {}
        self.lib = native.lib()
        self.nloci = int(nloci)
        species_names: List[str] = []
        sp_id: Dict[str, int] = {}
        sol = np.zeros(index.n_loci, dtype=np.int32)
        for l, (sp, _g) in enumerate(index.locus_names):
            if sp not in sp_id:
                sp_id[sp] = len(species_names)
                species_names.append(sp)
            sol[l] = sp_id[sp]
        self.species_names = species_names
        gdb = np.zeros(len(species_names), dtype=np.int32)
        for sp, i in sp_id.items():
            gdb[i] = (genes_in_db or {}).get(sp, int((sol == i).sum()))
        if db_ascii is None:
            seqs = [dbseq_of(t).encode("latin-1") for t in range(n_ref)]
            db_off = np.zeros(n_ref + 1, dtype=np.int64)
            db_off[1:] = np.cumsum([len(x) for x in seqs])
            db_ascii = np.frombuffer(b"".join(seqs), dtype=np.uint8)
        self.bad_len = np.asarray(streams.ref_lens, dtype=np.int64) > (db_off[1:] - db_off[:-1])
        t32 = lambda a: torch.from_numpy(np.ascontiguousarray(a)).to(dev)
        self.allele_num = t32(np.asarray([int(a) for a in index.allele], dtype=np.int64).astype(np.uint32).view(np.int32))
        self.species_of_locus = t32(sol)
        self.genes_in_db = t32(gdb)
        self.ref_len_d = t32(np.asarray(streams.ref_lens, dtype=np.int32))
        self.contig_start_d = torch.zeros(n_ref + 1, dtype=torch.int64, device=dev)
        self.max_chunks = 0
        self.rebind(streams)
        self.db_ascii_d = t32(np.concatenate([db_ascii, np.zeros(8, np.uint8)]))
        self.db_off_d = t32(np.asarray(db_off, dtype=np.int64))
        nl = index.n_loci
        self.scratch = torch.zeros(nl * 12 + 64, dtype=torch.uint8, device=dev)
        order = np.argsort(index.locus_of, kind="stable").astype(np.uint32)
        self.locus_rows = None if np.array_equal(order, np.arange(order.shape[0], dtype=order.dtype)) else t32(order.view(np.int32))
        self.locus_start = t32(np.searchsorted(index.locus_of[order], np.arange(nl + 1)).astype(np.int32))
        self.o_hdr, self.o_tid, self.o_sp, self.o_col, self.o_holes, self.o_snps = 0, 16, 16 + nl, 16 + 2 * nl, 17 + 3 * nl, 17 + 4 * nl
        self.o_first = 17 + 5 * nl
        self.n_small = (17 + 6 * nl + 7) // 4 * 4
        self.out = torch.zeros((self.n_small * 4 + self.max_cols + 16 + 15) // 16 * 16, dtype=torch.uint8, device=dev)
        self.small = self.out[: self.n_small * 4].view(torch.int32)
        self.cons = self.out[self.n_small * 4:]
        self.holes = self.small[self.o_holes:self.o_holes + nl]
        self.snps = self.small[self.o_snps:self.o_snps + nl]
        self.db_start_d = torch.zeros(nl + 1, dtype=torch.int64, device=dev)
        self.out_bytes = int(self.out.shape[0])
        if self.owner:
            self.out_all = torch.zeros(self.world * self.out_bytes + 16, dtype=torch.uint8, device=dev)
            self.out_h = torch.zeros(self.world * self.out_bytes + 16, dtype=torch.uint8).pin_memory()
            if self.p2p:
                self._init_p2p()
        else:
            self.out_h = torch.zeros(self.out_bytes, dtype=torch.uint8).pin_memory()
        self.small_h = self.out_h[: self.n_small * 4].view(torch.int32)
        self.cons_h = self.out_h[self.n_small * 4: self.out_bytes]
        self.genes_in_db_h = gdb
        self.ticket = torch.zeros(nl + 8, dtype=torch.int32, device=dev)
        self.fused_tail = os.environ.get("MMLST_FUSED_TAIL", "0") == "1"
        self.want_tables = False
        self._tables_h = None
        self._clean = False
        self.timers: Optional[Dict[str, list]] = None
        self.launches = 0

    def rebind(self, streams):
        if list(streams.ref_names) != self.index.ref_names or not np.array_equal(np.asarray(streams.ref_lens), np.asarray(self.s.ref_lens)):
            raise ValueError("rebind: the sample was aligned against a different reference set")
        self.s = streams
        self.use_runs = getattr(streams, "run_tid", None) is not None if self._use_runs_arg is None else bool(self._use_runs_arg)
        self.use_qc = self.use_runs and getattr(streams, "chunk_qlen", None) is not None
        self.idx_base = int(self._idx_base_arg) if self._idx_base_arg else int(getattr(streams, "idx_base", 0) or 0)
        self.contig_start_d.copy_(torch.from_numpy(np.asarray(streams.contig_start, dtype=np.uint64).view(np.int64)), non_blocking=False)
        need = int(streams.n_prec) // 512 + self.index.n_loci + 8
        if need > self.max_chunks:
            self.max_chunks = need
            self.chunks_d = torch.zeros(self.max_chunks * 8, dtype=torch.int32, device=self.dev)
        self.graph = None

    def _timed(self, name: str, fn):
        if self.timers is None:
            fn()
            return
        a, b = torch.cuda.Event(enable_timing=True), torch.cuda.Event(enable_timing=True)
        a.record()
        fn()
        b.record()
        self.timers.setdefault(name, []).append((a, b))

    def _stream(self):
        return torch.cuda.current_stream(self.dev).cuda_stream

    def reset_tables(self):
        self.zblock.zero_(); self.first_idx.fill_(-1); self.scratch.zero_(); self.ticket.zero_()
        self._clean = True

    def _score_call(self):
        s = self.s
        n = int(s.as0.shape[0])
        oi = native.ptr(getattr(s, "orig_idx", None))
        if n == 0:
            return
        if self.use_runs and self.use_qc:
            native.check(self.lib.mmlst_score_runs_qc_dev(native.ptr(s.run_tid), native.ptr(s.run_start), int(s.run_tid.shape[0]), native.ptr(s.chunk_run),
                                                          native.ptr(s.chunk_qlen), native.ptr(s.as0), native.ptr(s.xm3), oi, n, self.idx_base,
                                                          native.ptr(self.allow), self.n_ref, self.minscore, self.max_xM, self.min_read_len,
                                                          native.ptr(self.sum_as), native.ptr(self.n_hit), native.ptr(self.first_idx),
                                                          native.ptr(self.counters), self._stream()))
        elif self.use_runs:
            native.check(self.lib.mmlst_score_runs_dev(native.ptr(s.run_tid), native.ptr(s.run_start), int(s.run_tid.shape[0]), native.ptr(s.chunk_run),
                                                       native.ptr(s.as0), native.ptr(s.xm3), native.ptr(s.qlen), oi, n, self.idx_base,
                                                       native.ptr(self.allow), self.n_ref, self.minscore, self.max_xM, self.min_read_len,
                                                       native.ptr(self.sum_as), native.ptr(self.n_hit), native.ptr(self.first_idx),
                                                       native.ptr(self.counters), self._stream()))
        else:
            native.check(self.lib.mmlst_score_dev(native.ptr(s.tid), native.ptr(s.as0), native.ptr(s.xm3), native.ptr(s.qlen), oi, n, self.idx_base,
                                                  native.ptr(self.allow), native.ptr(self.locus_of), self.n_ref, self.minscore, self.max_xM,
                                                  self.min_read_len, native.ptr(self.sum_as), native.ptr(self.n_hit), native.ptr(self.first_idx),
                                                  native.ptr(self.counters), self._stream()))

    def run_score(self, reset: bool = True):
        s = self.s
        if reset:
            self.reset_tables()
        self._clean = False
        self._timed("score", self._score_call)
        self.launches += 1
        if self.dist and not self.owner:
            dist.allreduce_score_block(self.zscore, self.first_idx, self.group)

    def run_coverage(self, timed: bool = False):
        s = self.s
        if getattr(s, "qhash", None) is None:
            raise ValueError("streams were packed without QNAME keys (want_qhash)")
        n = int(s.tid.shape[0])
        slots = int(self.lib.mmlst_coverage_table_slots(n))
        if getattr(self, "_cov_table", None) is None or self._cov_table.shape[0] < slots * 3:
            self._cov_table = torch.empty(slots * 3, dtype=torch.int64, device=self.dev)
            self._cov = torch.zeros(self.index.n_loci, dtype=torch.int64, device=self.dev)
        ev = [torch.cuda.Event(enable_timing=True) for _ in range(3)]
        ev[0].record()
        self._cov_table[: slots * 3].zero_(); self._cov.zero_()
        ev[1].record()
        native.check(self.lib.mmlst_coverage_dev(native.ptr(s.tid), native.ptr(s.as0), native.ptr(s.xm3), native.ptr(s.qlen), 0, native.ptr(s.qhash),
                                                 n, self.idx_base, native.ptr(self.allow), native.ptr(self.locus_of), self.n_ref, self.minscore,
                                                 self.max_xM, self.min_read_len, native.ptr(self._cov_table), slots, native.ptr(self._cov),
                                                 self._stream()))
        ev[2].record()
        self.launches += 2
        if self.dist:
            torch.distributed.all_reduce(self._cov, group=self.group)
        cov = self._cov.cpu().numpy()
        out = {sp + "_" + g: int(cov[l]) for l, (sp, g) in enumerate(self.index.locus_names) if cov[l]}
        if timed:
            return out, {"memset_ms": ev[0].elapsed_time(ev[1]), "kernels_ms": ev[1].elapsed_time(ev[2]), "table_bytes": slots * 24}
        return out

    def select(self):
        sum_as = self.sum_as.cpu().numpy()
        n_hit = self.n_hit.cpu().numpy().view(np.uint32)
        first = self.first_idx.cpu().numpy().view(np.uint32)
        return api.fast_select(self.index, sum_as, n_hit, first, self.penalty), (sum_as, n_hit, first)

    def _db_for(self, tids: Tuple[int, ...]):
        hit = self._db_cache.get(tids)
        if hit is None:
            lens = [int(self.s.ref_lens[t]) for t in tids]
            col_off = np.zeros(len(tids) + 1, dtype=np.uint32)
            col_off[1:] = np.cumsum(lens)
            db = np.zeros(int(col_off[-1]) + 8, dtype=np.uint8)
            for i, t in enumerate(tids):
                sq = self.dbseq_of(t)
                if len(sq) < lens[i]:
                    raise IndexError("string index out of range: BAM LN > DB sequence length for %s" % self.index.ref_names[t])
                db[col_off[i]:col_off[i + 1]] = np.frombuffer(sq[:lens[i]].encode("latin-1"), dtype=np.uint8)
            hit = (col_off, torch.from_numpy(db).to(self.dev), torch.from_numpy(col_off.view(np.int32)).to(self.dev))
            if len(self._db_cache) > 64:
                self._db_cache.clear()
            self._db_cache[tids] = hit
        return hit

    def run_pileup_consensus(self, tids: Sequence[int]):
        tids = tuple(int(t) for t in tids)
        s = self.s
        col_off, db_d, col_off_d = self._db_for(tids)
        total = int(col_off[-1])
        chunks = build_chunks(s.contig_start, tids, col_off)
        self.counts[: total * 5].zero_()
        if chunks.shape[0]:
            chunks_d = torch.from_numpy(chunks.view(np.int32)).to(self.dev, non_blocking=True)
            def k():
                native.check(self.lib.mmlst_pileup_dev(native.ptr(s.p_recs), native.ptr(s.planes), native.ptr(chunks_d), int(chunks.shape[0]),
                                                       int(s.max_row_words), self.minscore, self.max_xM, native.ptr(self.counts), total,
                                                       self.impl, self._stream()))
            self._timed("pileup", k)
            self.launches += 1
        if self.dist:
            dist.allreduce_counts(self.counts[: total * 5], self.group)
        def k2():
            native.check(self.lib.mmlst_consensus_dev(native.ptr(self.counts), native.ptr(db_d), native.ptr(col_off_d), len(tids), self.mincov,
                                                      native.ptr(self.cons), native.ptr(self.holes), native.ptr(self.snps), self._stream()))
        self._timed("consensus", k2)
        self.launches += 1
        cons = self.cons[:total].cpu().numpy()
        holes = self.holes[: len(tids)].cpu().numpy()
        snps = self.snps[: len(tids)].cpu().numpy()
        return [cons[col_off[i]:col_off[i + 1]].tobytes().decode("latin-1") for i in range(len(tids))], holes, snps, col_off

    def _select_call(self, flags: int):
        sm, nl = self.small, self.index.n_loci
        base = sm.data_ptr()
        native.check(self.lib.mmlst_select_dev(native.ptr(self.sum_as), native.ptr(self.n_hit), native.ptr(self.first_idx), native.ptr(self.locus_rows),
                                               native.ptr(self.locus_start), native.ptr(self.allele_num), self.n_ref, native.ptr(self.species_of_locus),
                                               native.ptr(self.genes_in_db), nl, len(self.species_names), self.penalty, self.nloci,
                                               native.ptr(self.contig_start_d), native.ptr(self.ref_len_d), native.ptr(self.db_off_d),
                                               int(os.environ.get("MMLST_CHUNK_RECORDS", "0")),
                                               native.ptr(self.scratch), int(self.scratch.shape[0]), base + 4 * self.o_hdr, base + 4 * self.o_tid,
                                               base + 4 * self.o_sp, base + 4 * self.o_col, native.ptr(self.db_start_d), native.ptr(self.chunks_d),
                                               self.max_chunks, flags | (native.SELECT_LOCAL if self.owner else 0), native.ptr(self.counters),
                                               base + 4 * self.o_first, self._stream()))

    def _consensus_call(self, flags: int):
        nl = self.index.n_loci
        base = self.small.data_ptr()
        native.check(self.lib.mmlst_consensus_indirect_dev(native.ptr(self.counts), native.ptr(self.db_ascii_d), native.ptr(self.db_start_d),
                                                           base + 4 * self.o_col, nl, base + 4 * self.o_hdr, self.mincov, native.ptr(self.cons),
                                                           base + 4 * self.o_holes, base + 4 * self.o_snps, flags, self._stream()))

    def _pileup_call(self):
        s = self.s
        native.check(self.lib.mmlst_pileup_indirect_dev(native.ptr(s.p_recs), native.ptr(s.planes), native.ptr(self.chunks_d),
                                                        self.small.data_ptr() + 4 * self.o_hdr, int(s.max_row_words), self.minscore, self.max_xM,
                                                        native.ptr(self.counts), self.impl, self._stream()))

    def _pileup_consensus_call(self, flags: int):
        s, nl = self.s, self.index.n_loci
        base = self.small.data_ptr()
        native.check(self.lib.mmlst_pileup_consensus_indirect_dev(
            native.ptr(s.p_recs), native.ptr(s.planes), native.ptr(self.chunks_d), base + 4 * self.o_hdr, int(s.max_row_words), self.minscore, self.max_xM,
            native.ptr(self.counts), native.ptr(self.db_ascii_d), native.ptr(self.db_start_d), base + 4 * self.o_col, nl, self.mincov, native.ptr(self.cons),
            base + 4 * self.o_holes, base + 4 * self.o_snps, flags, native.ptr(self.ticket), self._stream()))

    def _enqueue(self):
        if not self._clean:
            self.reset_tables()
        self.run_score(reset=False)
        if self.want_tables:
            self._enqueue_tables()
        self._timed("select", lambda: self._select_call(native.SELECT_CONSUME | native.SELECT_SCRATCH_CLEAN))
        self.launches += 1
        if self.fused_tail and self.impl != 1 and not (self.dist and not self.owner):
            self._timed("pileup+consensus", lambda: self._pileup_consensus_call(native.CONSENSUS_CONSUME))
            self.launches += 1
        else:
            self._timed("pileup", self._pileup_call)
            self.launches += 1
            if self.dist and not self.owner:
                dist.allreduce_counts(self.counts, self.group)
            self._timed("consensus", lambda: self._consensus_call(native.CONSENSUS_CONSUME))
            self.launches += 1
        if self.p2p:
            native.check(self.lib.mmlst_xchg_publish_dev(native.ptr(self.out), self.out_bytes, native.ptr(self.peer_base), self.rank, self.world,
                                                         self.x_half, self.x_slot, self.x_flag_off, native.ptr(self.x_epoch), self._stream()))
            native.check(self.lib.mmlst_xchg_await_dev(native.ptr(self.xbuf), self.out_bytes, self.world, self.x_half, self.x_slot, self.x_flag_off,
                                                       native.ptr(self.out_all), native.ptr(self.x_epoch), native.ptr(self.x_ticket),
                                                       self.out_all.data_ptr() + self.world * self.out_bytes, self._stream()))
            self.launches += 2
            self.out_h.copy_(self.out_all, non_blocking=True)
        elif self.owner:
            torch.distributed.all_gather_into_tensor(self.out_all[: self.world * self.out_bytes], self.out, group=self.group)
            self.out_h.copy_(self.out_all, non_blocking=True)
        else:
            self.out_h.copy_(self.out, non_blocking=True)
        self._clean = True

    def time_kernels(self, reps: int = 20, alt: Optional["DevicePipeline"] = None, flush: Optional[torch.Tensor] = None) -> Dict[str, float]:
        pipes = [self] + ([alt] if alt is not None else [])
        for p in pipes:
            p.reset_tables()
            p.run_score(reset=False)
            p._select_call(native.SELECT_SCRATCH_CLEAN)
        torch.cuda.current_stream(self.dev).synchronize()
        out: Dict[str, float] = {}
        saved = [p.dist for p in pipes]
        for p in pipes:
            p.dist = False
        try:
            for name in ("select", "pileup", "consensus", "score"):
                for p in pipes:
                    p._launch_one(name)
                if name == "score" or flush is None:
                    a, b = torch.cuda.Event(enable_timing=True), torch.cuda.Event(enable_timing=True)
                    a.record()
                    for i in range(reps):
                        pipes[i % len(pipes)]._launch_one(name)
                    b.record()
                    b.synchronize()
                    out[name] = a.elapsed_time(b) / reps
                else:
                    pairs = []
                    for i in range(reps):
                        flush.zero_()
                        a, b = torch.cuda.Event(enable_timing=True), torch.cuda.Event(enable_timing=True)
                        a.record()
                        pipes[i % len(pipes)]._launch_one(name)
                        b.record()
                        pairs.append((a, b))
                    torch.cuda.current_stream(self.dev).synchronize()
                    out[name] = float(np.mean([a.elapsed_time(b) for a, b in pairs]))
        finally:
            for p, d in zip(pipes, saved):
                p.dist = d
                p._clean = False
        return out

    def time_score_variants(self, reps: int = 20, alt: Optional["DevicePipeline"] = None) -> Dict[str, float]:
        pipes = [self] + ([alt] if alt is not None else [])
        out: Dict[str, float] = {}
        want = None
        keys = ["0", "1", "2", "3", "4", "5", "2h", "3h", "4h", "5h"]
        if self.use_qc:
            keys += ["6", "6h", "6g10", "6g12"]
        grid0 = self.lib.mmlst_set_score_grid_scale(-1)
        for key in keys:
            v = int(key[0])
            self.lib.mmlst_set_score_variant(v)
            self.lib.mmlst_set_score_l2_hints(1 if key[1:2] == "h" else 0)
            self.lib.mmlst_set_score_grid_scale(int(key.split("g")[1]) if "g" in key else grid0)
            self.reset_tables()
            self._score_call()
            torch.cuda.current_stream(self.dev).synchronize()
            got = [self.zscore.clone(), self.first_idx.clone()]
            if want is None:
                want = got
            assert all(torch.equal(a, b) for a, b in zip(got, want)), "score kernel form %s disagrees with form 0" % key
            for p in pipes:
                p._score_call()
            a, b = torch.cuda.Event(enable_timing=True), torch.cuda.Event(enable_timing=True)
            a.record()
            for i in range(reps):
                pipes[i % len(pipes)]._score_call()
            b.record()
            b.synchronize()
            out[key] = a.elapsed_time(b) / reps
        self.lib.mmlst_set_score_grid_scale(grid0)
        for p in pipes:
            p._clean = False
        return out

    def time_score_half(self, reps: int = 20, alt: Optional["DevicePipeline"] = None) -> Dict[str, float]:
        pipes = [self] + ([alt] if alt is not None else [])
        out: Dict[str, float] = {}
        full = [p.s.as0 for p in pipes]
        n = int(self.s.as0.shape[0])
        try:
            for frac in (1, 2, 4):
                m = (n // frac) & ~255
                for p, f in zip(pipes, full):
                    p.s.as0 = f[:m]
                for p in pipes:
                    p._score_call()
                a, b = torch.cuda.Event(enable_timing=True), torch.cuda.Event(enable_timing=True)
                a.record()
                for i in range(reps):
                    pipes[i % len(pipes)]._score_call()
                b.record()
                b.synchronize()
                out["1/%d" % frac] = a.elapsed_time(b) / reps
        finally:
            for p, f in zip(pipes, full):
                p.s.as0 = f
                p._clean = False
        return out

    def _launch_one(self, name: str):
        s = self.s
        if name == "score":
            self._score_call()
        elif name == "select":
            self._select_call(native.SELECT_SCRATCH_CLEAN)
        elif name == "pileup":
            self._pileup_call()
        elif name == "consensus":
            self._consensus_call(0)
        else:
            raise ValueError(name)

    def _init_p2p(self):
        import torch.distributed._symmetric_memory as symm
        grp = self.group if self.group is not None else torch.distributed.group.WORLD
        self.rank = torch.distributed.get_rank(grp)
        self.x_slot = (self.out_bytes + 127) // 128 * 128
        self.x_half = self.world * self.x_slot
        self.x_flag_off = 2 * self.x_half
        self.xbuf = symm.empty(self.x_flag_off + 128 * ((8 * self.world + 127) // 128), dtype=torch.uint8, device=self.dev)
        self.xbuf.zero_()
        torch.cuda.synchronize(self.dev)
        self.xhdl = symm.rendezvous(self.xbuf, grp)
        ptrs = [int(x) for x in self.xhdl.buffer_ptrs]
        assert len(ptrs) == self.world and ptrs[self.rank] == self.xbuf.data_ptr(), "symmetric buffer: unexpected peer table"
        self.peer_base = torch.tensor(ptrs, dtype=torch.int64, device=self.dev)
        self.x_epoch = torch.zeros(1, dtype=torch.int64, device=self.dev)
        self.x_ticket = torch.zeros(1, dtype=torch.int32, device=self.dev)
        torch.cuda.synchronize(self.dev)
        torch.distributed.barrier(grp)

    def _finish_owner(self):
        nl = self.index.n_loci
        blocks, total, ignored = [], 0, 0
        if self.p2p and int(self.out_h[self.world * self.out_bytes:].view(torch.int32)[0]) != 0:
            raise RuntimeError("peer-memory exchange timed out waiting for a peer's result block")
        for r in range(self.world):
            blk = self.out_h[r * self.out_bytes:(r + 1) * self.out_bytes]
            h = blk[: self.n_small * 4].view(torch.int32).numpy()
            cons = blk[self.n_small * 4:].numpy()
            n = int(h[0])
            total += int(h[6:8].view(np.uint64)[0]); ignored += int(h[8:10].view(np.uint64)[0])
            if h[3] & 2:
                raise RuntimeError("chunk list overflow")
            tids = h[self.o_tid:self.o_tid + n]
            if self.bad_len[tids].any():
                raise IndexError("string index out of range: BAM LN > DB sequence length (metaMLST_functions.py:267)")
            col = h[self.o_col:self.o_col + n + 1]
            blocks.append({"tid": tids.tolist(), "species": h[self.o_sp:self.o_sp + n].tolist(),
                           "first": h[self.o_first:self.o_first + n].view(np.uint32).tolist(),
                           "payload": [(cons[col[i]:col[i + 1]].tobytes().decode("latin-1"), int(h[self.o_holes + i]), int(h[self.o_snps + i])) for i in range(n)]})
        self.total_reads, self.ignored_reads = total, ignored
        merged = dist.merge_owner_blocks(blocks, self.species_names, self.genes_in_db_h, self.nloci)
        return {sp: [(self.index.ref_names[t], seq, holes, snps) for t, (seq, holes, snps) in lst] for sp, lst in merged}

    def _finish(self):
        if self.owner:
            return self._finish_owner()
        h = self.small_h.numpy()
        n = int(h[0])
        self.total_reads = int(h[6:8].view(np.uint64)[0])
        self.ignored_reads = int(h[8:10].view(np.uint64)[0])
        if h[3] & 1:
            raise RuntimeError("Database is broken: a species has more detected loci than the genes table lists (metamlst.py:188)")
        if h[3] & 2:
            raise RuntimeError("chunk list overflow")
        tids = h[self.o_tid:self.o_tid + n]
        if self.bad_len[tids].any():
            raise IndexError("string index out of range: BAM LN > DB sequence length (metaMLST_functions.py:267)")
        col = h[self.o_col:self.o_col + n + 1]
        cons = self.cons_h.numpy()
        out: Dict[str, list] = {}
        for i in range(n):
            out.setdefault(self.species_names[int(h[self.o_sp + i])], []).append(
                (self.index.ref_names[int(tids[i])], cons[col[i]:col[i + 1]].tobytes().decode("latin-1"), int(h[self.o_holes + i]), int(h[self.o_snps + i])))
        return out

    def _enqueue_tables(self):
        if self._tables_h is None:
            self._tables_h = (torch.zeros(self.zscore.shape[0], dtype=torch.int64).pin_memory(), torch.zeros(self.n_ref, dtype=torch.int32).pin_memory())
        self._tables_h[0].copy_(self.zscore, non_blocking=True)
        self._tables_h[1].copy_(self.first_idx, non_blocking=True)

    def tables(self):
        z, f = self._tables_h
        n = self.n_ref
        return z[:n].numpy(), z[n + 2:].view(torch.int32)[:n].numpy().view(np.uint32), f.numpy().view(np.uint32)

    def step(self):
        self._enqueue()
        torch.cuda.current_stream(self.dev).synchronize()
        return self._finish()

    def capture(self):
        assert self.timers is None, "per-kernel timers are not capturable"
        self._enqueue()
        torch.cuda.synchronize(self.dev)
        n0 = self.launches
        self.graph = torch.cuda.CUDAGraph()
        with torch.cuda.graph(self.graph):
            self._enqueue()
        self.launches_per_step = self.launches - n0
        self.launches = n0

    def step_graph(self):
        if not self._clean:
            self.reset_tables()
        self.graph.replay()
        self.launches += self.launches_per_step
        torch.cuda.current_stream(self.dev).synchronize()
        return self._finish()

    def enqueue_step(self):
        if getattr(self, "graph", None) is not None:
            if not self._clean:
                self.reset_tables()
            self.graph.replay()
            self.launches += self.launches_per_step
        else:
            self._enqueue()

    def collect(self):
        torch.cuda.current_stream(self.dev).synchronize()
        return self._finish()

    def step_host_select(self):
        self.run_score()
        chosen, _raw = self.select()
        tids = [t for _sp, ts in chosen for t in ts]
        out: Dict[str, list] = {}
        if tids:
            seqs, holes, snps, _ = self.run_pileup_consensus(tids)
            i = 0
            for sp, ts in chosen:
                for t in ts:
                    out.setdefault(sp, []).append((self.index.ref_names[t], seqs[i], int(holes[i]), int(snps[i])))
                    i += 1
        return out


class CohortLanes:

    def __init__(self, make_pipe: Callable[[int], "DevicePipeline"], n_lanes: int = 2):
        self.pipes = [make_pipe(lane) for lane in range(n_lanes)]
        self.dev = self.pipes[0].dev
        self.streams = [torch.cuda.Stream(device=self.dev) for _ in range(n_lanes)]
        self.captured = False

    def warm_and_capture(self, graph: bool = True):
        res = []
        for p, st in zip(self.pipes, self.streams):
            with torch.cuda.stream(st):
                r = p.step()
                if graph:
                    p.capture()
                    assert p.step_graph() == r, "graph replay differs from the eager pass"
                res.append(r)
        self.captured = graph
        torch.cuda.synchronize(self.dev)
        return res

    def enqueue(self, i: int) -> None:
        lane = i % len(self.pipes)
        with torch.cuda.stream(self.streams[lane]):
            self.pipes[lane].enqueue_step()

    def fork(self, event: "torch.cuda.Event") -> None:
        for st in self.streams:
            st.wait_event(event)

    def join(self) -> None:
        cur = torch.cuda.current_stream(self.dev)
        for st in self.streams:
            ev = torch.cuda.Event()
            ev.record(st)
            cur.wait_event(ev)

    def collect(self):
        out = []
        for p, st in zip(self.pipes, self.streams):
            with torch.cuda.stream(st):
                out.append(p.collect())
        return out

    @property
    def launches(self) -> int:
        return sum(p.launches for p in self.pipes)


def device_select(index: api.AlleleIndex, sum_as: np.ndarray, n_hit: np.ndarray, first_idx: np.ndarray, penalty: int = 100,
                  nloci: int = 100, genes_in_db: Optional[Dict[str, int]] = None, device: str = "cuda:0"):
    lib = native.lib()
    dev = torch.device(device)
    n_ref, nl = len(index.ref_names), index.n_loci
    names: List[str] = []
    sid: Dict[str, int] = {}
    sol = np.zeros(nl, np.int32)
    for l, (sp, _g) in enumerate(index.locus_names):
        if sp not in sid:
            sid[sp] = len(names)
            names.append(sp)
        sol[l] = sid[sp]
    gdb = np.asarray([(genes_in_db or {}).get(sp, int((sol == i).sum())) for i, sp in enumerate(names)], np.int32)
    d = lambda a: torch.from_numpy(np.ascontiguousarray(a)).to(dev)
    t_sum, t_n, t_f = d(sum_as.astype(np.int64)), d(n_hit.astype(np.uint32).view(np.int32)), d(first_idx.astype(np.uint32).view(np.int32))
    order = np.argsort(index.locus_of, kind="stable").astype(np.uint32)
    identity = np.array_equal(order, np.arange(order.shape[0], dtype=order.dtype))
    t_rows, t_start = (None if identity else d(order.view(np.int32))), d(np.searchsorted(index.locus_of[order], np.arange(nl + 1)).astype(np.int32))
    t_an = d(np.asarray([int(a) for a in index.allele], np.int64).astype(np.uint32).view(np.int32))
    t_sol, t_gdb = d(sol), d(gdb)
    t_cs, t_rl, t_dbo = d(np.zeros(n_ref + 1, np.int64)), d(np.ones(n_ref, np.int32)), d(np.zeros(n_ref + 1, np.int64))
    scratch = torch.zeros(nl * 12 + 64, dtype=torch.uint8, device=dev)
    small = torch.zeros(16 + 3 * nl + 8, dtype=torch.int32, device=dev)
    dbs = torch.zeros(nl + 1, dtype=torch.int64, device=dev)
    chunks = torch.zeros(8 * (nl + 8), dtype=torch.int32, device=dev)
    base = small.data_ptr()
    native.check(lib.mmlst_select_dev(native.ptr(t_sum), native.ptr(t_n), native.ptr(t_f), native.ptr(t_rows), native.ptr(t_start), native.ptr(t_an),
                                      n_ref, native.ptr(t_sol), native.ptr(t_gdb), nl, len(names), int(penalty), int(nloci), native.ptr(t_cs),
                                      native.ptr(t_rl), native.ptr(t_dbo), 0, native.ptr(scratch), int(scratch.shape[0]), base,
                                      base + 4 * 16, base + 4 * (16 + nl), base + 4 * (16 + 2 * nl), native.ptr(dbs), native.ptr(chunks), nl + 8,
                                      0, 0, 0, torch.cuda.current_stream(dev).cuda_stream))
    h = small.cpu().numpy()
    n = int(h[0])
    out: Dict[str, List[int]] = {}
    for i in range(n):
        out.setdefault(names[int(h[16 + nl + i])], []).append(int(h[16 + i]))
    return list(out.items()), int(h[3])
```

metamlst_b200/streams.py:

```python
from __future__ import annotations

from typing import List, Optional

import numpy as np
import torch

from . import packing


class DeviceStreams:

    def __init__(self):
        self.ref_names: List[str] = []
        self.ref_lens: Optional[np.ndarray] = None

    def to_host(self, pinned: bool = True) -> packing.SoaHost:
        def h(t, dt):
            a = t.detach().cpu().numpy()
            return a.view(dt) if a.dtype != dt else a
        recs = self.p_recs.detach().cpu().numpy().reshape(-1).view(packing.PREC_DTYPE)
        oi = getattr(self, "orig_idx", None)
        soa = packing.SoaHost(self.ref_names, self.ref_lens, h(self.tid, np.uint32), h(self.as0, np.int16), h(self.xm3, np.uint8),
                              h(self.qlen, np.uint16), None if oi is None else h(oi, np.uint32), recs, h(self.planes, np.uint32),
                              int(self.max_row_words), self.contig_start.copy(), self.minqual, self.max_depth, self.n_dropped)
        if getattr(self, "run_tid", None) is not None:
            soa.run_tid, soa.run_start, soa.chunk_run = h(self.run_tid, np.uint32), h(self.run_start, np.uint32), h(self.chunk_run, np.uint32)
            if getattr(self, "chunk_qlen", None) is not None:
                soa.chunk_qlen = h(self.chunk_qlen, np.uint16)
        return soa.pin() if pinned else soa

    def build_runs(self) -> "DeviceStreams":
        n = int(self.tid.shape[0])
        self.run_tid = self.run_start = self.chunk_run = self.chunk_qlen = None
        if n == 0:
            return self
        assert n < 0xffffff00
        vals, counts = torch.unique_consecutive(self.tid, return_counts=True)
        start = torch.zeros(vals.shape[0] + 1, dtype=torch.int64, device=self.tid.device)
        start[1:] = torch.cumsum(counts, 0)
        first = torch.arange(0, n, 256, dtype=torch.int64, device=self.tid.device)
        self.chunk_run = (torch.searchsorted(start, first, right=True) - 1).to(torch.int32).contiguous()
        self.run_tid = vals.to(torch.int32).contiguous()
        self.run_start = start.to(torch.int32).contiguous()
        nc = (n + 255) // 256
        q = self.qlen.to(torch.int32)
        pad = torch.full((nc * 256 - n,), int(q[-1].item()), dtype=torch.int32, device=q.device)
        q2 = torch.cat([q, pad]).view(nc, 256)
        if bool((q2 == q2[:, :1]).all().item()):
            self.chunk_qlen = q2[:, 0].to(torch.int16).contiguous()
        return self

    def slice_ranges(self, rank: int, world: int) -> "DeviceStreams":
        if world <= 1:
            return self
        dev = self.as0.device
        n, P = int(self.tid.shape[0]), int(self.n_prec)
        a, b = (n * rank) // world, (n * (rank + 1)) // world
        p0, p1 = (P * rank) // world, (P * (rank + 1)) // world
        s = DeviceStreams()
        s.ref_names, s.ref_lens = self.ref_names, self.ref_lens
        s.minqual, s.max_depth, s.n_dropped = self.minqual, self.max_depth, getattr(self, "n_dropped", 0)
        s.tid, s.as0, s.xm3, s.qlen = self.tid[a:b].contiguous(), self.as0[a:b].contiguous(), self.xm3[a:b].contiguous(), self.qlen[a:b].contiguous()
        oi = getattr(self, "orig_idx", None)
        s.orig_idx = None if oi is None else oi[a:b].contiguous()
        s.idx_base = (int(getattr(self, "idx_base", 0) or 0) + a) if oi is None else 0
        qh = getattr(self, "qhash", None)
        s.qhash = None if qh is None else qh[a:b].contiguous()
        total_words = int(self.planes.shape[0]) - packing.PLANE_SLACK_WORDS
        off = lambda j: (int(self.p_recs[j, 1].item()) & 0xFFFFFFFF) if j < P else total_words
        w0, w1 = (off(p0), off(p1)) if p1 > p0 else (0, 0)
        recs = self.p_recs[p0:p1].clone()
        if w0 and p1 > p0:
            recs[:, 1] = ((recs[:, 1].to(torch.int64) & 0xFFFFFFFF) - w0).to(torch.int32)
        s.p_recs = recs
        s.planes = torch.cat([self.planes[w0:w1], torch.zeros(packing.PLANE_SLACK_WORDS, dtype=torch.int32, device=dev)])
        s.n_prec, s.max_row_words = p1 - p0, int(self.max_row_words)
        cs = np.asarray(self.contig_start, dtype=np.int64)
        s.contig_start = (np.clip(cs, p0, p1) - p0).astype(np.uint64)
        s.run_tid = s.run_start = s.chunk_run = s.chunk_qlen = None
        if getattr(self, "run_tid", None) is not None and b > a:
            s.build_runs()
            if int(s.run_tid.shape[0]) > 0.125 * (b - a):
                s.run_tid = s.run_start = s.chunk_run = s.chunk_qlen = None
        return s

    @classmethod
    def from_soa(cls, soa: packing.SoaHost, device, rank: int = 0, world: int = 1, mode: str = "ranges",
                 locus_of: Optional[np.ndarray] = None, want_qhash: bool = False, stream=None) -> "DeviceStreams":
        dev = torch.device(device)
        s = cls()
        s.ref_names = list(soa.ref_names)
        s.ref_lens = np.asarray(soa.ref_lens, dtype=np.int32)
        s.minqual, s.max_depth, s.n_dropped = int(soa.minqual), int(soa.max_depth or 0), int(soa.n_dropped_by_cap)
        n, P = soa.n_rec, soa.n_prec
        s.idx_base = 0
        s.orig_idx = None
        s.qhash = None

        def up(a, dt=None):
            a = np.ascontiguousarray(a)
            if dt is not None and a.dtype != dt:
                a = a.view(dt)
            t = torch.from_numpy(a)
            return t.to(dev, non_blocking=True)

        if world > 1 and mode not in ("ranges", "loci"):
            raise ValueError("mode must be 'ranges' or 'loci'")
        if world > 1 and mode == "loci":
            if locus_of is None:
                raise ValueError("mode='loci' needs locus_of[tid]")
            keep = (np.asarray(locus_of)[soa.tid] % world) == rank
            sel = np.nonzero(keep)[0]
            tid, as0, xm3, qlen = soa.tid[sel], soa.as0[sel], soa.xm3[sel], soa.qlen[sel]
            oi = (soa.orig_idx[sel] if soa.orig_idx is not None else sel).astype(np.uint32)
            p0, p1 = 0, P
            qh = soa.qhash[sel] if (want_qhash and soa.qhash is not None) else None
            whole_runs = False
        else:
            a, b = (n * rank) // world, (n * (rank + 1)) // world
            tid, as0, xm3, qlen = soa.tid[a:b], soa.as0[a:b], soa.xm3[a:b], soa.qlen[a:b]
            oi = soa.orig_idx[a:b] if soa.orig_idx is not None else None
            s.idx_base = a if oi is None else 0
            p0, p1 = (P * rank) // world, (P * (rank + 1)) // world
            qh = soa.qhash[a:b] if (want_qhash and soa.qhash is not None) else None
            whole_runs = world == 1
        s.tid, s.as0, s.xm3, s.qlen = up(tid, np.int32), up(as0), up(xm3), up(qlen, np.int16)
        if oi is not None:
            s.orig_idx = up(oi, np.int32)
        if qh is not None:
            s.qhash = up(qh, np.int64)
        recs = soa.p_recs[p0:p1]
        if p1 > p0:
            off = soa.p_row_off
            w0, w1 = int(off[p0]), int(off[p1])
            if w0:
                recs = recs.copy()
                recs["row_off"] -= np.uint32(w0)
            planes = soa.planes[w0:w1]
        else:
            planes = soa.planes[:0]
        s.p_recs = up(recs.view(np.int32).reshape(-1, 4)) if p1 > p0 else torch.zeros((0, 4), dtype=torch.int32, device=dev)
        s.planes = torch.cat([up(planes, np.int32), torch.zeros(packing.PLANE_SLACK_WORDS, dtype=torch.int32, device=dev)])
        s.n_prec = p1 - p0
        s.max_row_words = int(soa.max_row_words)
        cs = np.asarray(soa.contig_start, dtype=np.int64)
        s.contig_start = (np.clip(cs, p0, p1) - p0).astype(np.uint64)
        s.run_tid = s.run_start = s.chunk_run = s.chunk_qlen = None
        if whole_runs and soa.run_tid is not None:
            s.run_tid, s.run_start, s.chunk_run = up(soa.run_tid, np.int32), up(soa.run_start, np.int32), up(soa.chunk_run, np.int32)
            if soa.chunk_qlen is not None:
                s.chunk_qlen = up(soa.chunk_qlen, np.int16)
        elif soa.run_tid is not None and int(s.tid.shape[0]):
            s.build_runs()
            if int(s.run_tid.shape[0]) > 0.125 * int(s.tid.shape[0]):
                s.run_tid = s.run_start = s.chunk_run = s.chunk_qlen = None
        return s
```

Before: 1189 billion.

## Add packed 16-bit score words and SWAR/dp2a ring scoring kernel

At ingest, each read's alignment score (offset by a global bias) and mismatch count are packed into one 16-bit word, then validated against the span limit. A new default scoring variant streams these words through a shared-memory ring. It evaluates thresholds with SIMD-within-a-register arithmetic and accumulates scores with dp2a. This cuts the bytes read per record and the per-read instructions in the score stage. It costs an extra preprocessing pass and a 2-byte-per-read buffer, and falls back when the score range exceeds the word span.

```diff
diff --git a/include/mmlst.h b/include/mmlst.h
--- a/include/mmlst.h
+++ b/include/mmlst.h
@@ -55,8 +55,16 @@
                             uint64_t n_rec, uint64_t idx_base, const uint8_t* allow, uint32_t n_ref,
                             int minscore, int max_xm, int min_read_len,
                             int64_t* sum_as, uint32_t* n_hit, uint32_t* first_idx, uint64_t* counters, void* stream);
-#define MMLST_SCORE_VARIANT_DEFAULT 6
+int mmlst_score_words_dev(const int16_t* as0, const uint8_t* xm3, uint64_t n_rec, uint16_t* words, int32_t* bias, int32_t* valid,
+                          void* stream);
+int mmlst_score_runs_qcw_dev(const uint32_t* run_tid, const uint32_t* run_start, uint32_t n_runs, const uint32_t* chunk_run,
+                             const uint16_t* chunk_qlen, const uint16_t* words, int bias, const int16_t* as0, const uint8_t* xm3,
+                             const uint32_t* orig_idx, uint64_t n_rec, uint64_t idx_base, const uint8_t* allow, uint32_t n_ref,
+                             int minscore, int max_xm, int min_read_len,
+                             int64_t* sum_as, uint32_t* n_hit, uint32_t* first_idx, uint64_t* counters, void* stream);
+#define MMLST_SCORE_VARIANT_DEFAULT 7
 int mmlst_set_score_variant(int variant);
+int mmlst_score_last_form(void);
 #define MMLST_SCORE_L2_HINTS_DEFAULT 1
 int mmlst_set_score_l2_hints(int on);
 int mmlst_debug_timeline(uint64_t* dev_buf);
diff --git a/metamlst_b200/bam.py b/metamlst_b200/bam.py
--- a/metamlst_b200/bam.py
+++ b/metamlst_b200/bam.py
@@ -193,11 +193,14 @@
     s.planes = t(info.planes, int(info.n_plane_words), "<i4", torch.int32)
     s.n_prec, s.max_row_words = P, int(info.max_row_words)
     s.contig_start = _view(info.contig_start, n_ref + 1, np.uint64).copy()
-    s.run_tid = s.run_start = s.chunk_run = s.chunk_qlen = None
+    s.run_tid = s.run_start = s.chunk_run = s.chunk_qlen = s.score_w = s.score_w_bias = None
     if nr and nr <= 0.125 * n:
         s.run_tid, s.run_start = t(info.run_tid, nr, "<i4", torch.int32), t(info.run_start, nr + 1, "<i4", torch.int32)
         s.chunk_run = t(info.chunk_run, (n + 255) // 256, "<i4", torch.int32)
         s.chunk_qlen = t(info.chunk_qlen, (n + 255) // 256, "<i2", torch.int16) if info.chunk_qlen else None
+        if s.chunk_qlen is not None:
+            with torch.cuda.device(dev):
+                s.build_score_words()
     s.presorted = bool(info.presorted)
     s.ingest_seconds = dict(zip(("h2d", "inflate", "chain", "parse", "sort", "score_stream", "cap_compact", "pack"), [float(x) for x in info.seconds]))
     s.ingest_stats = {"bgzf_blocks": int(info.n_bgzf_blocks), "compressed_bytes": int(info.compressed_bytes), "inflated_bytes": int(info.inflated_bytes),
diff --git a/metamlst_b200/csrc/score_runs.cu b/metamlst_b200/csrc/score_runs.cu
--- a/metamlst_b200/csrc/score_runs.cu
+++ b/metamlst_b200/csrc/score_runs.cu
@@ -7,15 +7,18 @@
 static int score_variant() {
     if (g_score_variant < 0) {
         const char* e = getenv("MMLST_SCORE_VARIANT");
-        g_score_variant = (e && e[0] >= '0' && e[0] <= '6' && !e[1]) ? e[0] - '0' : MMLST_SCORE_VARIANT_DEFAULT;
+        g_score_variant = (e && e[0] >= '0' && e[0] <= '7' && !e[1]) ? e[0] - '0' : MMLST_SCORE_VARIANT_DEFAULT;
     }
     return g_score_variant;
 }
 extern "C" int mmlst_set_score_variant(int v) {
     const int prev = score_variant();
-    if (v >= 0 && v <= 6) g_score_variant = v;
+    if (v >= 0 && v <= 7) g_score_variant = v;
     return prev;
 }
+
+static thread_local int t_last_form = -1;
+extern "C" int mmlst_score_last_form(void) { return t_last_form; }
 
 static int g_score_l2_hints = -1;
 static int score_l2_hints() {
@@ -50,7 +53,7 @@
                              const int16_t* as0, const uint8_t* xm3, const uint16_t* qlen, const uint16_t* chunk_qlen, const uint32_t* orig_idx,
                              uint64_t n_rec, uint64_t idx_base, const uint8_t* allow, uint32_t n_ref, int minscore,
                              int max_xm, int min_read_len, int64_t* sum_as, uint32_t* n_hit, uint32_t* first_idx,
-                             uint64_t* counters, void* stream) {
+                             uint64_t* counters, void* stream, const uint16_t* words = nullptr, int bias = 0) {
     if (n_rec == 0) return MMLST_OK;
     if (!run_tid || !run_start || !chunk_run || !n_runs || !as0 || !xm3 || (!qlen && !chunk_qlen) || !allow || !sum_as || !n_hit || !first_idx || !counters) {
         mmlst_set_error("mmlst_score_runs_dev: null pointer");
@@ -63,13 +66,33 @@
         return MMLST_E_ARG;
     }
     RunArgs a{run_tid, run_start, chunk_run, n_runs, as0, xm3, qlen, orig_idx, chunk_qlen, n_rec, idx_base, allow, n_ref, minscore, max_xm,
-              min_read_len, reinterpret_cast<long long*>(sum_as), n_hit, first_idx, reinterpret_cast<unsigned long long*>(counters), score_l2_hints()};
+              min_read_len, reinterpret_cast<long long*>(sum_as), n_hit, first_idx, reinterpret_cast<unsigned long long*>(counters), score_l2_hints(),
+              words, bias};
     const uint64_t nchunks = n_rec >> 8;
     uint64_t want = (nchunks + 15) / 16;
     const int variant = score_variant();
     const cudaStream_t st = static_cast<cudaStream_t>(stream);
+    if (variant == 7 && words && chunk_qlen && !orig_idx && max_xm <= 14 && !(reinterpret_cast<uintptr_t>(words) & 15)) {
+        static int words_resident_by_device[MMLST_MAX_DEVICES] = {0};
+        int& words_resident = words_resident_by_device[mmlst_current_device()];
+        const size_t smem = (kThreads / 32) * static_cast<size_t>(kWordsNS) * (kWordsCH * 512u + sizeof(uint64_t));
+        if (!words_resident) {
+            CUDA_TRY(cudaFuncSetAttribute(score_runs_ring_words_kernel<>, cudaFuncAttributeMaxDynamicSharedMemorySize, static_cast<int>(smem)));
+            CUDA_TRY(cudaFuncSetAttribute(score_runs_ring_words_kernel<>, cudaFuncAttributePreferredSharedMemoryCarveout, cudaSharedmemCarveoutMaxShared));
+            int r = 0;
+            if (cudaOccupancyMaxActiveBlocksPerMultiprocessor(&r, score_runs_ring_words_kernel<>, kThreads, smem) != cudaSuccess || r < 1) r = 1;
+            words_resident = r;
+        }
+        const uint64_t cap = static_cast<uint64_t>(mmlst_num_sms()) * words_resident * score_grid8() / 8;
+        if (want > cap) want = cap;
+        if (want < 1) want = 1;
+        score_runs_ring_words_kernel<><<<static_cast<unsigned>(want), kThreads, smem, st>>>(a);
+        CUDA_TRY(cudaGetLastError());
+        t_last_form = 7;
+        return MMLST_OK;
+    }
     const bool tma_ok = !orig_idx && !(reinterpret_cast<uintptr_t>(xm3) & 15);
-    if (variant == 6 && tma_ok && chunk_qlen) {
+    if (variant >= 6 && tma_ok && chunk_qlen) {
         static int pair_resident_by_device[MMLST_MAX_DEVICES] = {0};
         int& pair_resident = pair_resident_by_device[mmlst_current_device()];
         const size_t smem = (kThreads / 32) * 2u * (4u * 768u + sizeof(uint64_t));
@@ -85,6 +108,7 @@
         if (want < 1) want = 1;
         score_runs_ring_pair_kernel<<<static_cast<unsigned>(want), kThreads, smem, st>>>(a);
         CUDA_TRY(cudaGetLastError());
+        t_last_form = 6;
         return MMLST_OK;
     }
     if (variant >= 2 && tma_ok) {
@@ -92,7 +116,7 @@
         int (&ring_resident)[4][8] = ring_resident_by_device[mmlst_current_device()];
         const int hint = a.l2_hints ? 1 : 0;
         const int q = (chunk_qlen ? 1 : 0) + 2 * hint;
-        const int rv = variant == 6 ? 5 : variant;
+        const int rv = variant >= 6 ? 5 : variant;
         const RingCfg cfg = chunk_qlen ? (hint ? ring_config<true, true>(rv) : ring_config<true, false>(rv))
                                        : (hint ? ring_config<false, true>(rv) : ring_config<false, false>(rv));
         const size_t smem = (kThreads / 32) * static_cast<size_t>(cfg.ns) * (cfg.ch * (chunk_qlen ? 768u : 1280u) + sizeof(uint64_t));
@@ -108,6 +132,7 @@
         if (want < 1) want = 1;
         cfg.kern<<<static_cast<unsigned>(want), kThreads, smem, st>>>(a);
         CUDA_TRY(cudaGetLastError());
+        t_last_form = rv;
         return MMLST_OK;
     }
     static int resident_by_device[MMLST_MAX_DEVICES][8] = {{0}};
@@ -126,6 +151,7 @@
     if (want < 1) want = 1;
     kern<<<static_cast<unsigned>(want), kThreads, 0, st>>>(a);
     CUDA_TRY(cudaGetLastError());
+    t_last_form = variant == 1 ? 1 : 0;
     return MMLST_OK;
 }
 
@@ -147,6 +173,37 @@
     if (n_rec && !chunk_qlen) { mmlst_set_error("mmlst_score_runs_qc_dev: null pointer"); return MMLST_E_ARG; }
     return score_runs_launch(run_tid, run_start, n_runs, chunk_run, as0, xm3, nullptr, chunk_qlen, orig_idx, n_rec, idx_base, allow, n_ref,
                              minscore, max_xm, min_read_len, sum_as, n_hit, first_idx, counters, stream);
+}
+
+extern "C" int mmlst_score_runs_qcw_dev(const uint32_t* run_tid, const uint32_t* run_start, uint32_t n_runs, const uint32_t* chunk_run,
+                                        const uint16_t* chunk_qlen, const uint16_t* words, int bias, const int16_t* as0, const uint8_t* xm3,
+                                        const uint32_t* orig_idx, uint64_t n_rec, uint64_t idx_base, const uint8_t* allow, uint32_t n_ref,
+                                        int minscore, int max_xm, int min_read_len, int64_t* sum_as, uint32_t* n_hit, uint32_t* first_idx,
+                                        uint64_t* counters, void* stream) {
+    if (n_rec && !chunk_qlen) { mmlst_set_error("mmlst_score_runs_qcw_dev: null pointer"); return MMLST_E_ARG; }
+    return score_runs_launch(run_tid, run_start, n_runs, chunk_run, as0, xm3, nullptr, chunk_qlen, orig_idx, n_rec, idx_base, allow, n_ref,
+                             minscore, max_xm, min_read_len, sum_as, n_hit, first_idx, counters, stream, words, bias);
+}
+
+extern "C" int mmlst_score_words_dev(const int16_t* as0, const uint8_t* xm3, uint64_t n_rec, uint16_t* words, int32_t* bias, int32_t* valid,
+                                     void* stream) {
+    if (!bias || !valid || (n_rec && (!as0 || !xm3 || !words))) { mmlst_set_error("mmlst_score_words_dev: null pointer"); return MMLST_E_ARG; }
+    const cudaStream_t st = static_cast<cudaStream_t>(stream);
+    CUDA_TRY(cudaMemsetAsync(bias, 0xff, sizeof(int32_t), st));
+    CUDA_TRY(cudaMemsetAsync(valid, 0xff, sizeof(int32_t), st));
+    if (n_rec) {
+        uint64_t blocks = (n_rec + 255) / 256;
+        const uint64_t cap = static_cast<uint64_t>(mmlst_num_sms()) * 8;
+        if (blocks > cap) blocks = cap;
+        uint32_t* const lo = reinterpret_cast<uint32_t*>(bias);
+        score_words_minmax_kernel<<<static_cast<unsigned>(blocks), 256, 0, st>>>(as0, n_rec, lo, reinterpret_cast<uint32_t*>(valid));
+        CUDA_TRY(cudaGetLastError());
+        score_words_kernel<<<static_cast<unsigned>(blocks), 256, 0, st>>>(as0, xm3, n_rec, lo, words);
+        CUDA_TRY(cudaGetLastError());
+    }
+    score_words_finish_kernel<<<1, 1, 0, st>>>(bias, valid);
+    CUDA_TRY(cudaGetLastError());
+    return MMLST_OK;
 }
 
 extern "C" int mmlst_expand_chunk_qlen_dev(const uint16_t* chunk_qlen, uint64_t n_rec, uint16_t* qlen, void* stream) {
diff --git a/metamlst_b200/csrc/score_runs_kernels.cuh b/metamlst_b200/csrc/score_runs_kernels.cuh
--- a/metamlst_b200/csrc/score_runs_kernels.cuh
+++ b/metamlst_b200/csrc/score_runs_kernels.cuh
@@ -15,6 +15,7 @@
     int minscore, max_xm, min_read_len;
     long long* sum_as; uint32_t* n_hit; uint32_t* first_idx; unsigned long long* counters;
     int l2_hints;
+    const uint16_t* words; int bias;
 };
 
 __device__ __forceinline__ void flush_run(const RunArgs& a, uint32_t key, long long s, uint32_t c, uint32_t mn) {
@@ -579,6 +580,261 @@
     }
 }
 
+constexpr int kWordSpan = 4095;
+
+__host__ __device__ __forceinline__ uint16_t score_word(int as0, uint32_t xm3, int bias) {
+    const int d = as0 - bias;
+    return static_cast<uint16_t>((static_cast<uint32_t>(d < kWordSpan ? d : kWordSpan) << 4) | (xm3 < 15u ? xm3 : 15u));
+}
+
+struct LoadedW { uint4 w8; uint32_t cq; };
+
+struct ThrW {
+    uint32_t as_T, as_TL;
+    uint32_t xm_T;
+    uint32_t h8;
+};
+
+__device__ __forceinline__ ThrW make_thr_w(const RunArgs& a) {
+    ThrW t;
+    const long long d = static_cast<long long>(a.minscore) - a.bias;
+    const bool none = d > kWordSpan || a.min_read_len > 65535 || a.max_xm < 0;
+    const uint32_t ts = (d <= 0 || none) ? 0u : static_cast<uint32_t>(d) << 4;
+    t.as_T = ts | (ts << 16); t.as_TL = t.as_T & ~H16;
+    t.xm_T = (0x10u | static_cast<uint32_t>(min(max(a.max_xm, 0), 14))) * 0x10001u;
+    t.h8 = none ? 0u : H8;
+    return t;
+}
+
+__device__ __forceinline__ void lane_pass_w(const LoadedW& L, const ThrW& t, int min_read_len, uint32_t& p_lo, uint32_t& p_hi) {
+    const uint32_t ww[4] = {L.w8.x, L.w8.y, L.w8.z, L.w8.w};
+    uint32_t m[4];
+#pragma unroll
+    for (int k = 0; k < 4; ++k) {
+        const uint32_t d = (ww[k] | H16) - t.as_TL;
+        const uint32_t ga = (ww[k] & ~t.as_T) | (~(ww[k] ^ t.as_T) & d);
+        const uint32_t gx = t.xm_T - (ww[k] & 0x000f000fu);
+        m[k] = ga & (gx << 11);
+    }
+    p_lo = (__byte_perm(m[0], m[1], 0x7531) & t.h8) >> 7;
+    p_hi = (__byte_perm(m[2], m[3], 0x7531) & t.h8) >> 7;
+    if (static_cast<int>(L.cq) < min_read_len) { p_lo = 0; p_hi = 0; }
+}
+
+#ifdef MMLST_HOST_EMUL
+inline uint32_t dp2a_lo_u(uint32_t a, uint32_t b, uint32_t c) { return c + (a & 0xffffu) * (b & 0xffu) + (a >> 16) * ((b >> 8) & 0xffu); }
+inline uint32_t dp2a_hi_u(uint32_t a, uint32_t b, uint32_t c) { return c + (a & 0xffffu) * ((b >> 16) & 0xffu) + (a >> 16) * (b >> 24); }
+#else
+__device__ __forceinline__ uint32_t dp2a_lo_u(uint32_t a, uint32_t b, uint32_t c) { return __dp2a_lo(a, b, c); }
+__device__ __forceinline__ uint32_t dp2a_hi_u(uint32_t a, uint32_t b, uint32_t c) { return __dp2a_hi(a, b, c); }
+#endif
+
+__device__ __forceinline__ uint32_t lane_wsum(const LoadedW& L, uint32_t p_lo, uint32_t p_hi, uint32_t s) {
+    constexpr uint32_t M = 0xfff0fff0u;
+    s = dp2a_lo_u(L.w8.x & M, p_lo, s);
+    s = dp2a_hi_u(L.w8.y & M, p_lo, s);
+    s = dp2a_lo_u(L.w8.z & M, p_hi, s);
+    return dp2a_hi_u(L.w8.w & M, p_hi, s);
+}
+
+__device__ __forceinline__ void add_words(const RunArgs& a, WarpRunPF& w, uint32_t ws, uint32_t c) {
+    w.s += static_cast<long long>(ws >> 4) + static_cast<long long>(a.bias) * c;
+    w.c += c;
+}
+
+__device__ __forceinline__ void reduce_chunk_w(const RunArgs& a, const ThrW& thr, WarpRunPF& w, const LoadedW& L, uint32_t base, uint32_t lane,
+                                               uint32_t& tot, uint32_t& ign) {
+    constexpr uint32_t R = 8;
+    const uint32_t idx0 = static_cast<uint32_t>(a.idx_base) + base + (lane << 3);
+    uint32_t p_lo, p_hi;
+    lane_pass_w(L, thr, a.min_read_len, p_lo, p_hi);
+    const uint32_t chunk_end = base + 256u;
+    if (chunk_end <= w.end) {
+        if (w.al) {
+            const uint32_t c = __popc(p_lo | (p_hi << 1));
+            tot += R;
+            ign += R - c;
+            add_words(a, w, __reduce_add_sync(FULL, lane_wsum(L, p_lo, p_hi, 0u)), __reduce_add_sync(FULL, c));
+            if (w.mn == 0xffffffffu) w.mn = __reduce_min_sync(FULL, first_pass_index(p_lo, p_hi, idx0));
+        }
+        if (chunk_end == w.end) next_run_pf<false>(a, w, lane, 0ull);
+        return;
+    }
+    const int lane0 = static_cast<int>(lane << 3);
+    uint32_t lo = base;
+    while (lo < chunk_end) {
+        const uint32_t hi = min(w.end, chunk_end);
+        if (w.al) {
+            const uint32_t klo = static_cast<uint32_t>(min(max(static_cast<int>(lo - base) - lane0, 0), 8));
+            const uint32_t khi = static_cast<uint32_t>(min(max(static_cast<int>(hi - base) - lane0, 0), 8));
+            uint32_t in_lo, in_hi;
+            segment_masks(klo, khi, in_lo, in_hi);
+            const uint32_t c = __popc((p_lo & in_lo) | ((p_hi & in_hi) << 1));
+            const uint32_t in = khi - klo;
+            tot += in;
+            ign += in - c;
+            add_words(a, w, __reduce_add_sync(FULL, lane_wsum(L, p_lo & in_lo, p_hi & in_hi, 0u)), __reduce_add_sync(FULL, c));
+            if (w.mn == 0xffffffffu) w.mn = __reduce_min_sync(FULL, first_pass_index(p_lo & in_lo, p_hi & in_hi, idx0));
+        }
+        if (hi == w.end) next_run_pf<false>(a, w, lane, 0ull);
+        lo = hi;
+    }
+}
+
+__device__ __forceinline__ void reduce_pair_w(const RunArgs& a, const ThrW& thr, WarpRunPF& w, const LoadedW& La, const LoadedW& Lb, uint32_t base,
+                                              uint32_t lane, uint32_t& tot, uint32_t& ign) {
+    if (base + 512u > w.end) {
+        reduce_chunk_w(a, thr, w, La, base, lane, tot, ign);
+        reduce_chunk_w(a, thr, w, Lb, base + 256u, lane, tot, ign);
+        return;
+    }
+    if (w.al) {
+        uint32_t pa_lo, pa_hi, pb_lo, pb_hi;
+        lane_pass_w(La, thr, a.min_read_len, pa_lo, pa_hi);
+        lane_pass_w(Lb, thr, a.min_read_len, pb_lo, pb_hi);
+        const uint32_t s = lane_wsum(Lb, pb_lo, pb_hi, lane_wsum(La, pa_lo, pa_hi, 0u));
+        const uint32_t c = __popc(pa_lo | (pa_hi << 1) | (pb_lo << 2) | (pb_hi << 3));
+        tot += 16u;
+        ign += 16u - c;
+        add_words(a, w, __reduce_add_sync(FULL, s), __reduce_add_sync(FULL, c));
+        if (w.mn == 0xffffffffu) {
+            const uint32_t idx0 = static_cast<uint32_t>(a.idx_base) + base + (lane << 3);
+            const uint32_t ma = first_pass_index(pa_lo, pa_hi, idx0);
+            w.mn = __reduce_min_sync(FULL, ma != 0xffffffffu ? ma : first_pass_index(pb_lo, pb_hi, idx0 + 256u));
+        }
+    }
+    if (base + 512u == w.end) next_run_pf<false>(a, w, lane, 0ull);
+}
+
+__device__ __forceinline__ void score_tail_w(const RunArgs& a, uint64_t nchunks, uint32_t lane, uint32_t& tot, uint32_t& ign) {
+    uint32_t r = __ldg(a.chunk_run + nchunks);
+    for (uint64_t i = (nchunks << 8) + lane; i < a.n_rec; i += 32) {
+        while (r + 1 < a.n_runs && i >= a.run_start[r + 1]) ++r;
+        const uint32_t key = a.run_tid[r];
+        if (!((key < a.n_ref) && a.allow[key])) continue;
+        ++tot;
+        const uint32_t wd = a.words[i];
+        const int as = static_cast<int>(wd >> 4) + a.bias;
+        if ((as >= a.minscore) && (int(a.chunk_qlen[nchunks]) >= a.min_read_len) && (static_cast<int>(wd & 15u) <= a.max_xm)) {
+            flush_run(a, key, as, 1u, static_cast<uint32_t>(a.idx_base + i));
+        } else {
+            ++ign;
+        }
+    }
+}
+
+constexpr int kWordsNS = 2, kWordsCH = 4;
+template <int NS = kWordsNS, int CH = kWordsCH>
+__global__ void __launch_bounds__(kThreads, 4) score_runs_ring_words_kernel(const RunArgs a) {
+    pdl_launch_dependents();
+    extern __shared__ __align__(128) uint8_t ring_raw[];
+    static_assert(CH % 2 == 0, "chunks are reduced in pairs");
+    constexpr uint32_t STAGE_B = CH * 512u;
+    constexpr int NW = kThreads / 32;
+    const uint32_t lane = threadIdx.x & 31u, wid = threadIdx.x >> 5;
+    uint8_t* const my = ring_raw + wid * (NS * STAGE_B);
+    uint64_t* const bars = reinterpret_cast<uint64_t*>(ring_raw + NW * NS * STAGE_B) + wid * NS;
+    if (threadIdx.x == 0) {
+        uint64_t* all = reinterpret_cast<uint64_t*>(ring_raw + NW * NS * STAGE_B);
+        for (int i = 0; i < NW * NS; ++i) mbar_init(all + i, 1);
+        fence_mbar_init();
+    }
+    __syncthreads();
+
+    const uint64_t warp = (static_cast<uint64_t>(blockIdx.x) * blockDim.x + threadIdx.x) >> 5;
+    const uint64_t nwarps = (static_cast<uint64_t>(gridDim.x) * blockDim.x) >> 5;
+    const uint64_t nchunks = a.n_rec >> 8;
+    const uint64_t per = (nchunks + nwarps - 1) / nwarps;
+    const uint64_t c0 = warp * per;
+    const uint64_t c1 = (c0 + per < nchunks) ? c0 + per : nchunks;
+    uint32_t tot = 0, ign = 0;
+    const ThrW thr = make_thr_w(a);
+
+    if (c0 < c1) {
+        const uint32_t ngroups = static_cast<uint32_t>((c1 - c0 + CH - 1) / CH);
+        auto issue = [&](uint32_t g, int stage) {
+            const uint64_t ch = c0 + static_cast<uint64_t>(g) * CH;
+            const uint32_t nch = (c1 - ch < static_cast<uint64_t>(CH)) ? static_cast<uint32_t>(c1 - ch) : static_cast<uint32_t>(CH);
+            uint8_t* st = my + stage * STAGE_B;
+            mbar_expect_tx(bars + stage, nch * 512u);
+            if (a.l2_hints) bulk_g2s_hint(st, a.words + (ch << 8), nch * 512u, bars + stage, l2_policy(1));
+            else bulk_g2s(st, a.words + (ch << 8), nch * 512u, bars + stage);
+        };
+        if (lane == 0) {
+            const uint32_t pre = ngroups < static_cast<uint32_t>(NS) ? ngroups : static_cast<uint32_t>(NS);
+            for (uint32_t g = 0; g < pre; ++g) issue(g, static_cast<int>(g));
+        }
+        WarpRunPF w;
+        open_run_pf<false>(a, w, __ldg(a.chunk_run + c0), 0ull);
+        uint32_t phase = 0;
+        int stage = 0;
+        auto load = [&](const uint8_t* st, uint32_t k, uint64_t ch) {
+            LoadedW L;
+            L.w8 = *reinterpret_cast<const uint4*>(st + k * 512u + lane * 16u);
+            L.cq = __ldg(a.chunk_qlen + ch + k);
+            return L;
+        };
+        for (uint32_t g = 0; g < ngroups; ++g) {
+            const uint64_t ch = c0 + static_cast<uint64_t>(g) * CH;
+            const uint32_t nch = (c1 - ch < static_cast<uint64_t>(CH)) ? static_cast<uint32_t>(c1 - ch) : static_cast<uint32_t>(CH);
+            mbar_wait(bars + stage, (phase >> stage) & 1u);
+            phase ^= 1u << stage;
+            const uint8_t* st = my + stage * STAGE_B;
+#pragma unroll
+            for (uint32_t k = 0; k < static_cast<uint32_t>(CH); k += 2) {
+                if (k < nch) {
+                    const bool two = k + 1u < nch;
+                    const LoadedW La = load(st, k, ch);
+                    LoadedW Lb = La;
+                    if (two) Lb = load(st, k + 1u, ch);
+                    if (k + 2u >= nch) {
+                        __syncwarp();
+                        if (lane == 0 && g + NS < ngroups) issue(g + NS, stage);
+                    }
+                    const uint32_t base = static_cast<uint32_t>((ch + k) << 8);
+                    if (two) reduce_pair_w(a, thr, w, La, Lb, base, lane, tot, ign);
+                    else reduce_chunk_w(a, thr, w, La, base, lane, tot, ign);
+                }
+            }
+            stage = (stage + 1 == NS) ? 0 : stage + 1;
+        }
+        if (lane == 0 && w.al) flush_run(a, w.key, w.s, w.c, w.mn);
+    }
+
+    if (warp == nwarps - 1 && (a.n_rec & 255u)) score_tail_w(a, nchunks, lane, tot, ign);
+    tot = __reduce_add_sync(FULL, tot);
+    ign = __reduce_add_sync(FULL, ign);
+    if (lane == 0 && tot) {
+        atomicAdd(a.counters + 0, static_cast<unsigned long long>(tot));
+        atomicAdd(a.counters + 1, static_cast<unsigned long long>(ign));
+    }
+}
+
+__global__ void __launch_bounds__(256) score_words_minmax_kernel(const int16_t* __restrict__ as0, uint64_t n, uint32_t* lo_p, uint32_t* nhi_p) {
+    const uint64_t stride = static_cast<uint64_t>(gridDim.x) * blockDim.x;
+    uint32_t lo = 0xffffffffu, hi = 0u;
+    for (uint64_t i = static_cast<uint64_t>(blockIdx.x) * blockDim.x + threadIdx.x; i < n; i += stride) {
+        const uint32_t v = static_cast<uint32_t>(as0[i] + 32768);
+        lo = min(lo, v);
+        hi = max(hi, v);
+    }
+    lo = __reduce_min_sync(FULL, lo);
+    hi = __reduce_max_sync(FULL, hi);
+    if ((threadIdx.x & 31u) == 0 && lo <= hi) { atomicMin(lo_p, lo); atomicMin(nhi_p, ~hi); }
+}
+__global__ void __launch_bounds__(256) score_words_kernel(const int16_t* __restrict__ as0, const uint8_t* __restrict__ xm3, uint64_t n,
+                                                          const uint32_t* lo_p, uint16_t* __restrict__ words) {
+    const int bias = static_cast<int>(*lo_p) - 32768;
+    const uint64_t stride = static_cast<uint64_t>(gridDim.x) * blockDim.x;
+    for (uint64_t i = static_cast<uint64_t>(blockIdx.x) * blockDim.x + threadIdx.x; i < n; i += stride) words[i] = score_word(as0[i], xm3[i], bias);
+}
+__global__ void score_words_finish_kernel(int32_t* bias, int32_t* valid) {
+    const uint32_t lo = static_cast<uint32_t>(*bias), hi = ~static_cast<uint32_t>(*valid);
+    const bool any = lo <= hi;
+    *bias = any ? static_cast<int32_t>(lo) - 32768 : 0;
+    *valid = !any || hi - lo <= static_cast<uint32_t>(kWordSpan);
+}
+
 struct RingCfg { void (*kern)(const RunArgs); uint32_t ch, ns; };
 template <bool QC, bool HINT>
 inline RingCfg ring_config(int variant) {
diff --git a/metamlst_b200/native.py b/metamlst_b200/native.py
--- a/metamlst_b200/native.py
+++ b/metamlst_b200/native.py
@@ -82,6 +82,10 @@
     "mmlst_chunk_qlen": (C.c_int, [C.c_void_p, C.c_uint64, C.c_void_p, C.POINTER(C.c_int)]),
     "mmlst_score_runs_qc_dev": (C.c_int, [C.c_void_p, C.c_void_p, C.c_uint32] + [C.c_void_p] * 5 + [C.c_uint64, C.c_uint64, C.c_void_p, C.c_uint32,
                                           C.c_int, C.c_int, C.c_int, C.c_void_p, C.c_void_p, C.c_void_p, C.c_void_p, C.c_void_p]),
+    "mmlst_score_words_dev": (C.c_int, [C.c_void_p, C.c_void_p, C.c_uint64, C.c_void_p, C.c_void_p, C.c_void_p, C.c_void_p]),
+    "mmlst_score_runs_qcw_dev": (C.c_int, [C.c_void_p, C.c_void_p, C.c_uint32] + [C.c_void_p] * 3 + [C.c_int] + [C.c_void_p] * 3 +
+                                 [C.c_uint64, C.c_uint64, C.c_void_p, C.c_uint32, C.c_int, C.c_int, C.c_int] + [C.c_void_p] * 5),
+    "mmlst_score_last_form": (C.c_int, []),
     "mmlst_expand_chunk_qlen_dev": (C.c_int, [C.c_void_p, C.c_uint64, C.c_void_p, C.c_void_p]),
     "mmlst_inflate_raw": (C.c_int, [C.c_void_p, C.c_size_t, C.c_void_p, C.c_size_t, C.POINTER(C.c_size_t)]),
     "mmlst_set_score_variant": (C.c_int, [C.c_int]),
diff --git a/metamlst_b200/pipeline.py b/metamlst_b200/pipeline.py
--- a/metamlst_b200/pipeline.py
+++ b/metamlst_b200/pipeline.py
@@ -43,6 +43,7 @@
         self.dev = dev
         self.use_runs = bool(use_runs) if use_runs is not None else getattr(streams, "run_tid", None) is not None
         self.use_qc = self.use_runs and getattr(streams, "chunk_qlen", None) is not None
+        self.score_form = None
         n_ref = len(index.ref_names)
         self.n_ref = n_ref
         self.allow = torch.from_numpy(index.allow_mask(species_filter)).to(dev)
@@ -157,7 +158,14 @@
         oi = native.ptr(getattr(s, "orig_idx", None))
         if n == 0:
             return
-        if self.use_runs and self.use_qc:
+        words = getattr(s, "score_w", None) if self.use_runs and self.use_qc else None
+        if words is not None:
+            native.check(self.lib.mmlst_score_runs_qcw_dev(native.ptr(s.run_tid), native.ptr(s.run_start), int(s.run_tid.shape[0]), native.ptr(s.chunk_run),
+                                                           native.ptr(s.chunk_qlen), native.ptr(words), int(s.score_w_bias), native.ptr(s.as0),
+                                                           native.ptr(s.xm3), oi, n, self.idx_base, native.ptr(self.allow), self.n_ref, self.minscore,
+                                                           self.max_xM, self.min_read_len, native.ptr(self.sum_as), native.ptr(self.n_hit),
+                                                           native.ptr(self.first_idx), native.ptr(self.counters), self._stream()))
+        elif self.use_runs and self.use_qc:
             native.check(self.lib.mmlst_score_runs_qc_dev(native.ptr(s.run_tid), native.ptr(s.run_start), int(s.run_tid.shape[0]), native.ptr(s.chunk_run),
                                                           native.ptr(s.chunk_qlen), native.ptr(s.as0), native.ptr(s.xm3), oi, n, self.idx_base,
                                                           native.ptr(self.allow), self.n_ref, self.minscore, self.max_xM, self.min_read_len,
@@ -174,6 +182,7 @@
                                                   native.ptr(self.allow), native.ptr(self.locus_of), self.n_ref, self.minscore, self.max_xM,
                                                   self.min_read_len, native.ptr(self.sum_as), native.ptr(self.n_hit), native.ptr(self.first_idx),
                                                   native.ptr(self.counters), self._stream()))
+        self.score_form = int(self.lib.mmlst_score_last_form()) if self.use_runs else None
 
     def run_score(self, reset: bool = True):
         s = self.s
@@ -377,6 +386,8 @@
         keys = ["0", "1", "2", "3", "4", "5", "2h", "3h", "4h", "5h"]
         if self.use_qc:
             keys += ["6", "6h", "6g10", "6g12"]
+            if getattr(self.s, "score_w", None) is not None:
+                keys += ["7", "7h"]
         grid0 = self.lib.mmlst_set_score_grid_scale(-1)
         for key in keys:
             v = int(key[0])
diff --git a/metamlst_b200/streams.py b/metamlst_b200/streams.py
--- a/metamlst_b200/streams.py
+++ b/metamlst_b200/streams.py
@@ -5,7 +5,7 @@
 import numpy as np
 import torch
 
-from . import packing
+from . import native, packing
 
 
 class DeviceStreams:
@@ -31,7 +31,7 @@
 
     def build_runs(self) -> "DeviceStreams":
         n = int(self.tid.shape[0])
-        self.run_tid = self.run_start = self.chunk_run = self.chunk_qlen = None
+        self.run_tid = self.run_start = self.chunk_run = self.chunk_qlen = self.score_w = self.score_w_bias = None
         if n == 0:
             return self
         assert n < 0xffffff00
@@ -48,6 +48,23 @@
         q2 = torch.cat([q, pad]).view(nc, 256)
         if bool((q2 == q2[:, :1]).all().item()):
             self.chunk_qlen = q2[:, 0].to(torch.int16).contiguous()
+            self.build_score_words()
+        return self
+
+    def build_score_words(self) -> "DeviceStreams":
+        self.score_w = self.score_w_bias = None
+        if getattr(self, "chunk_qlen", None) is None or self.as0.device.type != "cuda":
+            return self
+        dev = self.as0.device
+        n = int(self.as0.shape[0])
+        as0, xm3 = self.as0.contiguous(), self.xm3.contiguous()
+        words = torch.empty(n, dtype=torch.int16, device=dev)
+        bv = torch.empty(2, dtype=torch.int32, device=dev)
+        native.check(native.lib().mmlst_score_words_dev(as0.data_ptr(), xm3.data_ptr(), n, words.data_ptr(), bv.data_ptr(), bv.data_ptr() + 4,
+                                                        torch.cuda.current_stream(dev).cuda_stream))
+        bias, valid = (int(x) for x in bv.tolist())
+        if valid:
+            self.score_w, self.score_w_bias = words, bias
         return self
 
     def slice_ranges(self, rank: int, world: int) -> "DeviceStreams":
@@ -77,11 +94,11 @@
         s.n_prec, s.max_row_words = p1 - p0, int(self.max_row_words)
         cs = np.asarray(self.contig_start, dtype=np.int64)
         s.contig_start = (np.clip(cs, p0, p1) - p0).astype(np.uint64)
-        s.run_tid = s.run_start = s.chunk_run = s.chunk_qlen = None
+        s.run_tid = s.run_start = s.chunk_run = s.chunk_qlen = s.score_w = s.score_w_bias = None
         if getattr(self, "run_tid", None) is not None and b > a:
             s.build_runs()
             if int(s.run_tid.shape[0]) > 0.125 * (b - a):
-                s.run_tid = s.run_start = s.chunk_run = s.chunk_qlen = None
+                s.run_tid = s.run_start = s.chunk_run = s.chunk_qlen = s.score_w = s.score_w_bias = None
         return s
 
     @classmethod
@@ -145,13 +162,15 @@
         s.max_row_words = int(soa.max_row_words)
         cs = np.asarray(soa.contig_start, dtype=np.int64)
         s.contig_start = (np.clip(cs, p0, p1) - p0).astype(np.uint64)
-        s.run_tid = s.run_start = s.chunk_run = s.chunk_qlen = None
+        s.run_tid = s.run_start = s.chunk_run = s.chunk_qlen = s.score_w = s.score_w_bias = None
         if whole_runs and soa.run_tid is not None:
             s.run_tid, s.run_start, s.chunk_run = up(soa.run_tid, np.int32), up(soa.run_start, np.int32), up(soa.chunk_run, np.int32)
             if soa.chunk_qlen is not None:
                 s.chunk_qlen = up(soa.chunk_qlen, np.int16)
+                if int(s.tid.shape[0]):
+                    s.build_score_words()
         elif soa.run_tid is not None and int(s.tid.shape[0]):
             s.build_runs()
             if int(s.run_tid.shape[0]) > 0.125 * int(s.tid.shape[0]):
-                s.run_tid = s.run_start = s.chunk_run = s.chunk_qlen = None
+                s.run_tid = s.run_start = s.chunk_run = s.chunk_qlen = s.score_w = s.score_w_bias = None
         return s
```

Measured after the change: 1209 billion (median of 6 runs). 1.6% higher.
